# LBM-EPFL/MaD

Measured on NVIDIA B200. Metric: voxels/sec scale-space+detect+describe(+match), higher is better.
Workload: dtype f32 grids, f64 line accumulation, u8 x u8 -> s32 matching

## Files before the change

include/mad_b200.h:

```cpp
#ifndef MAD_B200_H
#define MAD_B200_H

#include <stddef.h>
#include <stdint.h>

#ifdef __cplusplus
extern "C" {
#endif

#define MAD_OK 0
#define MAD_ERR_ARG (-1)
#define MAD_ERR_CUDA (-2)
#define MAD_ERR_CAPACITY (-3)
#define MAD_ERR_NODEVICE (-4)

#define MAD_MAX_ORI 36
#define MAD_DSC_LEN 1024
#define MAD_DSC_REFUSED (1 << 30)

typedef struct MadKeypoint {
    int32_t vox[3];
    int32_t oct;
    float off[3];
    float val;
    int32_t peak[3];
    int32_t accepted;
} MadKeypoint;

typedef struct MadOriented {
    int32_t kp;
    int16_t main_bin;
    int16_t sec_bin;
} MadOriented;

typedef struct MadZoneTable {
    int32_t n_zones;
    int32_t n_belts;
    const double* bounds;
    const int32_t* belt_first;
    const double* belt_phi;
    const void* fast;
} MadZoneTable;

#define MAD_ZONE_FAST_BYTES 2048
int mad_zone_fast_build(const MadZoneTable* zones_host, void* fast_out, void* stream);

const char* mad_last_error_string(void);
int mad_version(void);
int mad_device_info(int* sm_count, int* cc_major, int* cc_minor);

int mad_publish_small(const void* src_dev, void* dst_host_mapped, int bytes, void* stream);

int mad_copy_to_host(const void* src_dev, void* dst_host_mapped, long long bytes, int n_ctas, void* stream);

long long mad_launch_count(void);
int mad_profile_enable(int on);
int mad_profile_count(void);
int mad_profile_get(int i, const char** name, float* ms);
int mad_profile_reset(void);

int mad_grid_max(const float* grid, long long n, float* out_max_ord, void* stream);
float mad_grid_max_decode(unsigned int ord);
int mad_threshold_normalise(float* grid, long long n, float isovalue, float vmax, int divide, void* stream);
int mad_grid_bbox(const float* grid, int nx, int ny, int nz, int* bbox6, void* stream);
int mad_crop_pad3d(const float* in, int nx, int ny, int nz, int x0, int y0, int z0, int cx, int cy, int cz,
                   int pad, float* out, void* stream);

int mad_pad3d(const float* in, int nx, int ny, int nz, int pad, float* out, void* stream);

size_t mad_upsample_workspace_bytes(int bx, int by, int bz);
int mad_upsample_presmooth(const float* base, int bx, int by, int bz,
                           const double* gauss_w_host, int radius,
                           float* up, void* workspace, size_t workspace_bytes, void* stream);

size_t mad_log_gauss_workspace_bytes(int nx, int ny, int nz);
int mad_log_gauss(const float* grid, int nx, int ny, int nz,
                  const double* w0_host, const double* w2_host, int radius, float scale,
                  float* log_out, float* gauss_out, void* workspace, size_t workspace_bytes,
                  int exact_f64, void* stream);

int mad_gradient(const float* gauss, int nx, int ny, int nz, float* grad4, void* stream);
size_t mad_gradient_tiles(int nx, int ny, int nz);
int mad_gradient_mark(const MadKeypoint* kp, int n_kp, const int* dims_oct_host, int reach_oct0, int reach_oct1,
                      uint8_t* flags_oct0, uint8_t* flags_oct1, void* stream);
int mad_gradient_masked(const float* gauss, int nx, int ny, int nz, float* grad4, uint8_t* flags, void* stream);

int mad_detect(const float* log_grid, int nx, int ny, int nz, int oct, int border,
               float threshold, MadKeypoint* cand, int cap, int* count, void* stream);

size_t mad_sort_keypoints_workspace_bytes(int n);
int mad_sort_keypoints(const MadKeypoint* cand, int n, const int* dims_oct_host,
                       MadKeypoint* out, int* out_count,
                       void* workspace, size_t workspace_bytes, void* stream);

int mad_orient(const float* grad4_oct0, const float* grad4_oct1, const int* dims_oct_host,
               const MadKeypoint* kp, int n_kp, int r, const MadZoneTable* zones112_host,
               const double* r1_table, int lim_main, int lim_sec,
               int32_t* n_ori, int32_t* slots, void* stream);

size_t mad_compact_oriented_workspace_bytes(int n_kp);
int mad_compact_oriented(const int32_t* n_ori, const int32_t* slots, int n_kp,
                         MadOriented* oriented, int cap, int* out_count,
                         void* workspace, size_t workspace_bytes, void* stream);

int mad_describe(const float* grad4_oct0, const float* grad4_oct1, const int* dims_oct_host,
                 const MadKeypoint* kp, const MadOriented* oriented, int n_oriented, int r,
                 const MadZoneTable* zones16_host, const double* rf_table, const double* rf_inv_table,
                 int rf_zones, int16_t* dsc, void* stream);

typedef struct MadDscSet {
    const int16_t* dsc;
    const void* half;
    const int32_t* norm2;
    const uint8_t* u8;
    const float* rnorm;
    int32_t rows;
    int32_t rows_padded;
    int32_t max_entry;
    int32_t max_norm2;
} MadDscSet;

int mad_dsc_prepare(const int16_t* dsc, int rows, int rows_padded, int32_t* norm2, float* rnorm,
                    uint8_t* u8, int32_t* max_entry, int32_t* max_norm2, void* stream);
int mad_dsc_norms(const int16_t* dsc, int rows, int32_t* norm2, void* stream);
int mad_dsc_to_half(const int16_t* dsc, int rows, int rows_padded, void* half_out, void* stream);

int mad_match_segments(int M, int N, int impl);
int mad_match_count(const MadDscSet* hi, const MadDscSet* lo, double cc, int n_seg, int32_t* seg_count, int impl,
                    void* stream);
int mad_match_fill(const MadDscSet* hi, const MadDscSet* lo, double cc, int n_seg, const int64_t* seg_offset,
                   int32_t* pair_hi, int32_t* pair_lo, double* pair_score, int impl, void* stream);
size_t mad_exclusive_scan_workspace_bytes(int n);
int mad_exclusive_scan_i32_to_i64(const int32_t* in, int n, int64_t* out, int64_t* total,
                                  void* workspace, size_t workspace_bytes, void* stream);

int mad_match_pairs(const MadDscSet* hi, const MadDscSet* lo, double cc, uint64_t* cand_key, int32_t* cand_dot,
                    uint64_t cap, uint64_t* count, void* stream);
size_t mad_match_pairs_finish_workspace_bytes(long long n);
int mad_match_pairs_finish(const uint64_t* cand_key, const int32_t* cand_dot, long long n, int hi_rows, int lo_rows,
                           const int32_t* hi_n2, const int32_t* lo_n2, int32_t* pair_hi, int32_t* pair_lo,
                           double* pair_score, void* workspace, size_t workspace_bytes, void* stream);
int mad_match_pairs_finish_dot(const uint64_t* cand_key, const int32_t* cand_dot, long long n, int hi_rows, int lo_rows,
                               int32_t* pair_hi, int32_t* pair_lo, int32_t* pair_dot, void* workspace, size_t workspace_bytes,
                               void* stream);

size_t mad_match_topk_workspace_bytes(int M, int N, int k, int impl);
int mad_match_topk(const MadDscSet* hi, const MadDscSet* lo, int k, int lo_index_base,
                   int32_t* topk_idx, double* topk_score, void* workspace, size_t workspace_bytes,
                   int impl, void* stream);
#define MAD_TOPK_INCOMPLETE (-2)
int mad_topk_merge(const int32_t* idx_in, const double* score_in, int G, int M, int k,
                   int32_t* idx_out, double* score_out, void* stream);

int mad_mark_used(const int32_t* idx, long long n, uint8_t* used, void* stream);
int mad_repeatability(const int32_t* pair_hi, const int32_t* pair_lo, const double* pair_score, long long n_pairs,
                      const double* hi_subv, const double* lo_subv, const int32_t* hi_meta, const int32_t* lo_meta,
                      const double* rf_table, const double* rf_inv_table, int rf_zones,
                      const double* hi_cloud, int n_hi_cloud, const double* lo_sorted, const int32_t* cell_start,
                      const uint32_t* near_bits, const double* grid_org_host, const int* grid_dims_host,
                      double dist, double* results, void* stream);

int mad_density_splat(const double* xyz, const double* mass, int n_atoms, const double* min_host, double voxelsp,
                      int margin, int px, int py, int pz, double* grid, void* stream);
int mad_normalise_f64(double* grid, long long n, void* scratch8, void* stream);
int mad_conv_full_f64(const double* in, long long outer, int n, long long inner, const double* w_dev, int radius,
                      void* out, int out_is_f32, void* stream);

size_t mad_box_scores_workspace_bytes(int ex, int ey, int ez);
int mad_box_scores(const float* g1, int nx1, int ny1, int nz1, const float* g2, int nx2, int ny2, int nz2,
                   const int* box_host, float isovalue, double* out8, void* workspace, size_t workspace_bytes,
                   void* stream);
int mad_grid_count_gt(const float* grid, long long n, float thr, unsigned long long* out, void* stream);
int mad_mask_with(float* g1, int nx1, int ny1, int nz1, const float* g2, int nx2, int ny2, int nz2,
                  const int* shift_host, const int* lo_host, const int* hi_host, void* stream);
int mad_refine_rigid(const float* grad4, int nx, int ny, int nz, const double* px, const double* py, const double* pz,
                     double voxsp, const double* init, const double* center, const double* max_dist, int n_problems,
                     int n_atoms, int n_steps, double max_step, double min_step, double* coords_out, double* meta_out,
                     void* stream);

#ifdef __cplusplus
}
#endif
#endif
```

mad_b200/_lib.py:

```python
import ctypes as C
import os

import numpy as np

HERE = os.path.dirname(os.path.abspath(__file__))
LIB_PATH = os.path.join(HERE, "libmad_b200.so")


class MadError(RuntimeError):
    pass


if not os.path.exists(LIB_PATH):
    raise ImportError(
        "mad_b200: %s is missing -- build the CUDA library first (python -m mad_b200.build). "
        "There is no CPU fallback." % LIB_PATH)

lib = C.CDLL(LIB_PATH)

KEYPOINT_DTYPE = np.dtype([("vox", "<i4", 3), ("oct", "<i4"), ("off", "<f4", 3), ("val", "<f4"),
                           ("peak", "<i4", 3), ("accepted", "<i4")])
ORIENTED_DTYPE = np.dtype([("kp", "<i4"), ("main", "<i2"), ("sec", "<i2")])
assert KEYPOINT_DTYPE.itemsize == 48 and ORIENTED_DTYPE.itemsize == 8
MAX_ORI = 36
DSC_LEN = 1024
DSC_REFUSED = 1 << 30
TOPK_INCOMPLETE = -2
TOPK_MAX = 32
ZONE_FAST_BYTES = 2048


class MadZoneTable(C.Structure):
    _fields_ = [("n_zones", C.c_int32), ("n_belts", C.c_int32), ("bounds", C.c_void_p),
                ("belt_first", C.c_void_p), ("belt_phi", C.c_void_p), ("fast", C.c_void_p)]


class MadDscSet(C.Structure):
    _fields_ = [("dsc", C.c_void_p), ("half", C.c_void_p), ("norm2", C.c_void_p), ("u8", C.c_void_p),
                ("rnorm", C.c_void_p), ("rows", C.c_int32), ("rows_padded", C.c_int32), ("max_entry", C.c_int32),
                ("max_norm2", C.c_int32)]


_P = C.c_void_p
_I = C.c_int
_SZ = C.c_size_t

SIGNATURES = {
    "mad_last_error_string": (C.c_char_p, []),
    "mad_version": (_I, []),
    "mad_device_info": (_I, [C.POINTER(_I), C.POINTER(_I), C.POINTER(_I)]),
    "mad_launch_count": (C.c_longlong, []),
    "mad_profile_enable": (_I, [_I]),
    "mad_profile_count": (_I, []),
    "mad_profile_get": (_I, [_I, C.POINTER(C.c_char_p), C.POINTER(C.c_float)]),
    "mad_profile_reset": (_I, []),
    "mad_publish_small": (_I, [_P, _P, _I, _P]),
    "mad_copy_to_host": (_I, [_P, _P, C.c_longlong, _I, _P]),
    "mad_zone_fast_build": (_I, [C.POINTER(MadZoneTable), _P, _P]),
    "mad_grid_max": (_I, [_P, C.c_longlong, _P, _P]),
    "mad_grid_max_decode": (C.c_float, [C.c_uint]),
    "mad_threshold_normalise": (_I, [_P, C.c_longlong, C.c_float, C.c_float, _I, _P]),
    "mad_grid_bbox": (_I, [_P, _I, _I, _I, _P, _P]),
    "mad_crop_pad3d": (_I, [_P, _I, _I, _I, _I, _I, _I, _I, _I, _I, _I, _P, _P]),
    "mad_pad3d": (_I, [_P, _I, _I, _I, _I, _P, _P]),
    "mad_upsample_workspace_bytes": (_SZ, [_I, _I, _I]),
    "mad_upsample_presmooth": (_I, [_P, _I, _I, _I, _P, _I, _P, _P, _SZ, _P]),
    "mad_log_gauss_workspace_bytes": (_SZ, [_I, _I, _I]),
    "mad_log_gauss": (_I, [_P, _I, _I, _I, _P, _P, _I, C.c_float, _P, _P, _P, _SZ, _I, _P]),
    "mad_gradient": (_I, [_P, _I, _I, _I, _P, _P]),
    "mad_gradient_tiles": (_SZ, [_I, _I, _I]),
    "mad_gradient_mark": (_I, [_P, _I, _P, _I, _I, _P, _P, _P]),
    "mad_gradient_masked": (_I, [_P, _I, _I, _I, _P, _P, _P]),
    "mad_detect": (_I, [_P, _I, _I, _I, _I, _I, C.c_float, _P, _I, _P, _P]),
    "mad_sort_keypoints_workspace_bytes": (_SZ, [_I]),
    "mad_sort_keypoints": (_I, [_P, _I, _P, _P, _P, _P, _SZ, _P]),
    "mad_orient": (_I, [_P, _P, _P, _P, _I, _I, C.POINTER(MadZoneTable), _P, _I, _I, _P, _P, _P]),
    "mad_compact_oriented_workspace_bytes": (_SZ, [_I]),
    "mad_compact_oriented": (_I, [_P, _P, _I, _P, _I, _P, _P, _SZ, _P]),
    "mad_describe": (_I, [_P, _P, _P, _P, _P, _I, _I, C.POINTER(MadZoneTable), _P, _P, _I, _P, _P]),
    "mad_dsc_prepare": (_I, [_P, _I, _I, _P, _P, _P, _P, _P, _P]),
    "mad_match_pairs": (_I, [C.POINTER(MadDscSet), C.POINTER(MadDscSet), C.c_double, _P, _P, C.c_uint64, _P, _P]),
    "mad_match_pairs_finish_workspace_bytes": (_SZ, [C.c_longlong]),
    "mad_match_pairs_finish": (_I, [_P, _P, C.c_longlong, _I, _I, _P, _P, _P, _P, _P, _P, _SZ, _P]),
    "mad_match_pairs_finish_dot": (_I, [_P, _P, C.c_longlong, _I, _I, _P, _P, _P, _P, _SZ, _P]),
    "mad_dsc_norms": (_I, [_P, _I, _P, _P]),
    "mad_dsc_to_half": (_I, [_P, _I, _I, _P, _P]),
    "mad_match_segments": (_I, [_I, _I, _I]),
    "mad_match_count": (_I, [C.POINTER(MadDscSet), C.POINTER(MadDscSet), C.c_double, _I, _P, _I, _P]),
    "mad_match_fill": (_I, [C.POINTER(MadDscSet), C.POINTER(MadDscSet), C.c_double, _I, _P, _P, _P, _P, _I, _P]),
    "mad_exclusive_scan_workspace_bytes": (_SZ, [_I]),
    "mad_exclusive_scan_i32_to_i64": (_I, [_P, _I, _P, _P, _P, _SZ, _P]),
    "mad_match_topk_workspace_bytes": (_SZ, [_I, _I, _I, _I]),
    "mad_match_topk": (_I, [C.POINTER(MadDscSet), C.POINTER(MadDscSet), _I, _I, _P, _P, _P, _SZ, _I, _P]),
    "mad_topk_merge": (_I, [_P, _P, _I, _I, _I, _P, _P, _P]),
    "mad_density_splat": (_I, [_P, _P, _I, _P, C.c_double, _I, _I, _I, _I, _P, _P]),
    "mad_normalise_f64": (_I, [_P, C.c_longlong, _P, _P]),
    "mad_conv_full_f64": (_I, [_P, C.c_longlong, _I, C.c_longlong, _P, _I, _P, _I, _P]),
    "mad_mark_used": (_I, [_P, C.c_longlong, _P, _P]),
    "mad_repeatability": (_I, [_P, _P, _P, C.c_longlong, _P, _P, _P, _P, _P, _P, _I, _P, _I, _P, _P, _P, _P, _P,
                               C.c_double, _P, _P]),
    "mad_box_scores_workspace_bytes": (_SZ, [_I, _I, _I]),
    "mad_box_scores": (_I, [_P, _I, _I, _I, _P, _I, _I, _I, _P, C.c_float, _P, _P, _SZ, _P]),
    "mad_grid_count_gt": (_I, [_P, C.c_longlong, C.c_float, _P, _P]),
    "mad_mask_with": (_I, [_P, _I, _I, _I, _P, _I, _I, _I, _P, _P, _P, _P]),
    "mad_refine_rigid": (_I, [_P, _I, _I, _I, _P, _P, _P, C.c_double, _P, _P, _P, _I, _I, _I, C.c_double, C.c_double,
                              _P, _P, _P]),
}

for _name, (_res, _args) in SIGNATURES.items():
    _f = getattr(lib, _name)
    _f.restype = _res
    _f.argtypes = _args


def last_error():
    s = lib.mad_last_error_string()
    return s.decode() if s else ""


def check(rc, what):
    if rc != 0:
        raise MadError("%s failed with status %d: %s" % (what, rc, last_error()))


def call(name, *args):
    check(getattr(lib, name)(*args), name)
```

mad_b200/csrc/api.cu:

```cuda
#include <stdarg.h>
#include <string.h>

#include "common.cuh"
#include "match_common.cuh"

static thread_local char g_err[512] = "";

void mad_set_error(const char* fmt, ...) {
    va_list ap;
    va_start(ap, fmt);
    vsnprintf(g_err, sizeof(g_err), fmt, ap);
    va_end(ap);
}

int mad_sm_count() {
    static int cached = 0;
    if (!cached) {
        int dev = 0, n = 0;
        if (cudaGetDevice(&dev) == cudaSuccess &&
            cudaDeviceGetAttribute(&n, cudaDevAttrMultiProcessorCount, dev) == cudaSuccess && n > 0)
            cached = n;
        else
            return 148;
    }
    return cached;
}

#include <atomic>
#include <mutex>
#include <vector>
namespace {
struct ProfRec { const char* name; cudaEvent_t a, b; };
std::atomic<long long> g_launches{0};
std::atomic<int> g_prof_on{0};
std::mutex g_prof_mu;
std::vector<ProfRec> g_prof;
}

MadProfScope::MadProfScope(const char* name, cudaStream_t stream) : slot(-1), st(stream) {
    g_launches.fetch_add(1, std::memory_order_relaxed);
    if (!g_prof_on.load(std::memory_order_relaxed)) return;
    ProfRec r;
    r.name = name;
    if (cudaEventCreate(&r.a) != cudaSuccess || cudaEventCreate(&r.b) != cudaSuccess) return;
    cudaEventRecord(r.a, st);
    std::lock_guard<std::mutex> lk(g_prof_mu);
    g_prof.push_back(r);
    slot = (int)g_prof.size() - 1;
}
MadProfScope::~MadProfScope() {
    if (slot < 0) return;
    std::lock_guard<std::mutex> lk(g_prof_mu);
    cudaEventRecord(g_prof[slot].b, st);
}

extern "C" long long mad_launch_count(void) { return g_launches.load(); }
extern "C" int mad_profile_enable(int on) {
    g_prof_on.store(on ? 1 : 0);
    return MAD_OK;
}
extern "C" int mad_profile_count(void) {
    std::lock_guard<std::mutex> lk(g_prof_mu);
    return (int)g_prof.size();
}
extern "C" int mad_profile_get(int i, const char** name, float* ms) {
    std::lock_guard<std::mutex> lk(g_prof_mu);
    MAD_CHECK_ARG(name && ms && i >= 0 && i < (int)g_prof.size());
    MAD_CUDA(cudaEventSynchronize(g_prof[i].b));
    MAD_CUDA(cudaEventElapsedTime(ms, g_prof[i].a, g_prof[i].b));
    *name = g_prof[i].name;
    return MAD_OK;
}
extern "C" int mad_profile_reset(void) {
    std::lock_guard<std::mutex> lk(g_prof_mu);
    for (auto& r : g_prof) { cudaEventDestroy(r.a); cudaEventDestroy(r.b); }
    g_prof.clear();
    return MAD_OK;
}

extern "C" const char* mad_last_error_string(void) { return g_err; }
extern "C" int mad_version(void) { return 100; }

extern "C" int mad_device_info(int* sm_count, int* cc_major, int* cc_minor) {
    MAD_CHECK_ARG(sm_count && cc_major && cc_minor);
    int dev = 0;
    MAD_CUDA(cudaGetDevice(&dev));
    MAD_CUDA(cudaDeviceGetAttribute(sm_count, cudaDevAttrMultiProcessorCount, dev));
    MAD_CUDA(cudaDeviceGetAttribute(cc_major, cudaDevAttrComputeCapabilityMajor, dev));
    MAD_CUDA(cudaDeviceGetAttribute(cc_minor, cudaDevAttrComputeCapabilityMinor, dev));
    return MAD_OK;
}

int mad_check_descriptor_sets(const MadDscSet* hi, const MadDscSet* lo, const char* who) {
    if (hi->max_entry >= MAD_DSC_REFUSED || lo->max_entry >= MAD_DSC_REFUSED) {
        mad_set_error("%s: not a descriptor set (a negative entry, or a squared norm >= 2^31)", who);
        return MAD_ERR_ARG;
    }
    return MAD_OK;
}

static bool fp16_exact(const MadDscSet* hi, const MadDscSet* lo) {
    return hi->max_entry >= 0 && lo->max_entry >= 0 && hi->max_entry <= 2048 && lo->max_entry <= 2048 &&
           hi->max_norm2 >= 0 && lo->max_norm2 >= 0 && (double)hi->max_norm2 * (double)lo->max_norm2 <= 281474976710656.0;
}

static int check_sets(const MadDscSet* hi, const MadDscSet* lo, int impl) {
    MAD_CHECK_ARG(hi && lo && hi->rows >= 0 && lo->rows >= 0);
    MAD_CHECK_ARG(impl == 0 || impl == 1 || impl == 2);
    if (hi->rows == 0 || lo->rows == 0) return MAD_OK;
    MAD_CHECK_ARG(hi->norm2 && lo->norm2);
    const int rc = mad_check_descriptor_sets(hi, lo, "mad_match");
    if (rc != MAD_OK) return rc;
    if (impl == 1) {
        MAD_CHECK_ARG(hi->dsc && lo->dsc);
    } else {
        if (impl == 2) MAD_CHECK_ARG(hi->half && lo->half);
        if (impl == 2 && !fp16_exact(hi, lo)) {
            mad_set_error("mad_match: the fp16 kernel (impl = 2) is exact only for entries in [0, 2048] and max |hi|^2 * max "
                          "|lo|^2 <= 2^48 (here max entry %d / %d, max |.|^2 %d / %d; -1 = not known): use impl = 1",
                          hi->max_entry, lo->max_entry, hi->max_norm2, lo->max_norm2);
            return MAD_ERR_ARG;
        }
        if (impl == 0) MAD_CHECK_ARG(hi->u8 && lo->u8 && lo->rnorm);
        MAD_CHECK_ARG(hi->rows_padded >= hi->rows && hi->rows_padded % 128 == 0);
        MAD_CHECK_ARG(lo->rows_padded >= lo->rows && lo->rows_padded % 128 == 0);
        if (impl == 0 && (hi->max_entry > 255 || lo->max_entry > 255)) {
            mad_set_error("mad_match: descriptor entries up to %d do not fit the uint8 kernel (use impl = 2)",
                          hi->max_entry > lo->max_entry ? hi->max_entry : lo->max_entry);
            return MAD_ERR_ARG;
        }
    }
    return MAD_OK;
}

static int run_match(const MadDscSet* hi, const MadDscSet* lo, double cc, int mode, int S, int32_t* seg_count,
                     const int64_t* seg_offset, int32_t* pair_hi, int32_t* pair_lo, double* pair_score, int k, int base,
                     int32_t* topk_idx, double* topk_score, int impl, cudaStream_t st) {
    if (impl == 1)
        return mad_match_simt(hi->dsc, hi->rows, lo->dsc, lo->rows, hi->norm2, lo->norm2, cc, mode, S, seg_count, seg_offset,
                              pair_hi, pair_lo, pair_score, k, base, topk_idx, topk_score, st);
    return mad_match_tc(hi->half, hi->rows, hi->rows_padded, lo->half, lo->rows, lo->rows_padded, hi->norm2, lo->norm2, cc,
                        mode, S, seg_count, seg_offset, pair_hi, pair_lo, pair_score, k, base, topk_idx, topk_score, st);
}

extern "C" int mad_match_segments(int M, int N, int impl) {
    return impl == 0 ? mad_match_u8_segments(M, N) : mad_match_tc_segments(M, N);
}

static int check_segments(const MadDscSet* hi, const MadDscSet* lo, int n_seg) {
    const int n_tiles = (int)mad_ceil_div(lo->rows, 128);
    MAD_CHECK_ARG(n_seg >= 1 && n_seg <= (n_tiles > 0 ? n_tiles : 1));
    (void)hi;
    return MAD_OK;
}

extern "C" int mad_match_count(const MadDscSet* hi, const MadDscSet* lo, double cc, int n_seg, int32_t* seg_count,
                               int impl, void* stream) {
    if (impl == 0) {
        mad_set_error("%s: impl 0 (the one-pass uint8 tcgen05 kernel) has no count/fill form -- call mad_match_pairs + "
                      "mad_match_pairs_finish; count/fill serve impl 1 (SIMT check) and 2 (fp16 tcgen05)", "mad_match_count");
        return MAD_ERR_ARG;
    }
    int rc = check_sets(hi, lo, impl);
    if (rc != MAD_OK) return rc;
    if (hi->rows == 0) return MAD_OK;
    MAD_CHECK_ARG(seg_count && n_seg >= 1);
    if (lo->rows == 0) {
        MAD_CUDA(cudaMemsetAsync(seg_count, 0, sizeof(int32_t) * (size_t)hi->rows * n_seg, (cudaStream_t)stream));
        return MAD_OK;
    }
    rc = check_segments(hi, lo, n_seg);
    if (rc != MAD_OK) return rc;
    return run_match(hi, lo, cc, 0, n_seg, seg_count, nullptr, nullptr, nullptr, nullptr, 0, 0, nullptr, nullptr, impl,
                     (cudaStream_t)stream);
}

extern "C" int mad_match_fill(const MadDscSet* hi, const MadDscSet* lo, double cc, int n_seg, const int64_t* seg_offset,
                              int32_t* pair_hi, int32_t* pair_lo, double* pair_score, int impl, void* stream) {
    if (impl == 0) {
        mad_set_error("%s: impl 0 (the one-pass uint8 tcgen05 kernel) has no count/fill form -- call mad_match_pairs + "
                      "mad_match_pairs_finish; count/fill serve impl 1 (SIMT check) and 2 (fp16 tcgen05)", "mad_match_fill");
        return MAD_ERR_ARG;
    }
    int rc = check_sets(hi, lo, impl);
    if (rc != MAD_OK) return rc;
    if (hi->rows == 0 || lo->rows == 0) return MAD_OK;
    MAD_CHECK_ARG(seg_offset && pair_hi && pair_lo && pair_score);
    rc = check_segments(hi, lo, n_seg);
    if (rc != MAD_OK) return rc;
    return run_match(hi, lo, cc, 1, n_seg, nullptr, seg_offset, pair_hi, pair_lo, pair_score, 0, 0, nullptr, nullptr, impl,
                     (cudaStream_t)stream);
}

static int u8_lists_per_segment(int k) { return k <= 8 ? 3 : 2; }
static int topk_lists(int M, int N, int k, int impl) {
    return impl == 0 ? u8_lists_per_segment(k) * mad_match_u8_segments_topk(M, N) : mad_match_segments(M, N, impl);
}

static size_t topk_part_workspace_bytes(int M, int N, int k, int impl) {
    const int S = topk_lists(M, N, k, impl);
    if (S <= 1 || M <= 0) return 256;
    return mad_align_up((size_t)S * M * k * sizeof(int32_t), 256) + mad_align_up((size_t)S * M * k * sizeof(double), 256);
}

static int topk_tail_rows(int M, int k, int impl) {
    if (impl != 0 || k > 8 || getenv("MAD_TOPK_NO_TAIL")) return 0;
    const int per_wave = mad_sm_count() / 2;
    const int pairs = (int)mad_ceil_div(M, 256);
    if (per_wave <= 0 || pairs <= per_wave) return 0;
    const int tail = pairs % per_wave;
    if (tail == 0 || 2 * tail > per_wave) return 0;
    return M - (pairs - tail) * 256;
}

extern "C" size_t mad_match_topk_workspace_bytes(int M, int N, int k, int impl) {
    const int tail = topk_tail_rows(M, k, impl);
    if (tail <= 0) return topk_part_workspace_bytes(M, N, k, impl);
    return std::max(topk_part_workspace_bytes(M - tail, N, k, impl), topk_part_workspace_bytes(tail, N, k, impl));
}

static int topk_part(const MadDscSet* hi, const MadDscSet* lo, int k, int lo_index_base, int32_t* topk_idx, double* topk_score,
                     void* workspace, size_t workspace_bytes, int impl, cudaStream_t st) {
    const int M = hi->rows;
    const int S = topk_lists(M, lo->rows, k, impl);
    auto run_topk = [&](int lists, int32_t* oi, double* os) {
        const int segs = impl == 0 ? lists / u8_lists_per_segment(k) : lists;
        if (impl == 0)
            return mad_match_u8_topk(hi->u8, hi->rows, hi->rows_padded, lo->u8, lo->rows, lo->rows_padded, hi->norm2,
                                     lo->norm2, lo->rnorm, segs, k, lo_index_base, oi, os, st);
        return run_match(hi, lo, 0.0, 2, segs, nullptr, nullptr, nullptr, nullptr, nullptr, k, lo_index_base, oi, os, impl, st);
    };
    if (S == 1) return run_topk(1, topk_idx, topk_score);
    MAD_CHECK_ARG(workspace && workspace_bytes >= topk_part_workspace_bytes(M, lo->rows, k, impl));
    int32_t* pidx = reinterpret_cast<int32_t*>(workspace);
    double* pscore = reinterpret_cast<double*>(reinterpret_cast<char*>(workspace) +
                                               mad_align_up((size_t)S * M * k * sizeof(int32_t), 256));
    int rc = run_topk(S, pidx, pscore);
    if (rc != MAD_OK) return rc;
    return mad_topk_merge_launch(pidx, pscore, S, M, k, topk_idx, topk_score, st);
}

extern "C" int mad_match_topk(const MadDscSet* hi, const MadDscSet* lo, int k, int lo_index_base, int32_t* topk_idx,
                              double* topk_score, void* workspace, size_t workspace_bytes, int impl, void* stream) {
    int rc = check_sets(hi, lo, impl);
    if (rc != MAD_OK) return rc;
    MAD_CHECK_ARG(k >= 1 && k <= MAD_TOPK_MAX);
    if (hi->rows == 0) return MAD_OK;
    MAD_CHECK_ARG(topk_idx && topk_score);
    cudaStream_t st = (cudaStream_t)stream;
    const int M = hi->rows;
    if (lo->rows == 0) {
        MAD_CUDA(cudaMemsetAsync(topk_idx, 0xFF, sizeof(int32_t) * (size_t)M * k, st));
        return mad_topk_merge_launch(topk_idx, topk_score, 0, M, k, topk_idx, topk_score, st);
    }
    const int tail = topk_tail_rows(M, k, impl);
    if (tail <= 0) return topk_part(hi, lo, k, lo_index_base, topk_idx, topk_score, workspace, workspace_bytes, impl, st);
    const int M0 = M - tail;
    MadDscSet a = *hi, b = *hi;
    a.rows = M0;
    a.rows_padded = M0;
    b.rows = tail;
    b.rows_padded = hi->rows_padded - M0;
    b.dsc = hi->dsc ? hi->dsc + (size_t)M0 * MAD_DSC_LEN : nullptr;
    b.u8 = hi->u8 ? hi->u8 + (size_t)M0 * MAD_DSC_LEN : nullptr;
    b.norm2 = hi->norm2 + M0;
    b.rnorm = hi->rnorm ? hi->rnorm + M0 : nullptr;
    rc = topk_part(&a, lo, k, lo_index_base, topk_idx, topk_score, workspace, workspace_bytes, impl, st);
    if (rc != MAD_OK) return rc;
    return topk_part(&b, lo, k, lo_index_base, topk_idx + (size_t)M0 * k, topk_score + (size_t)M0 * k, workspace, workspace_bytes,
                     impl, st);
}

namespace {
__global__ void publish_small_kernel(const unsigned int* __restrict__ src, volatile unsigned int* dst, int n_words) {
    for (int i = threadIdx.x; i < n_words; i += blockDim.x) dst[i] = src[i];
    __threadfence_system();
}
}

extern "C" int mad_publish_small(const void* src_dev, void* dst_host_mapped, int bytes, void* stream) {
    MAD_CHECK_ARG(src_dev && dst_host_mapped && bytes > 0 && bytes <= 4096 && bytes % 4 == 0);
    MAD_CHECK_ARG((reinterpret_cast<uintptr_t>(src_dev) & 3) == 0 && (reinterpret_cast<uintptr_t>(dst_host_mapped) & 3) == 0);
    MAD_PROF("publish_small_kernel", stream);
    publish_small_kernel<<<1, 64, 0, (cudaStream_t)stream>>>(static_cast<const unsigned int*>(src_dev),
                                                             static_cast<volatile unsigned int*>(dst_host_mapped), bytes / 4);
    MAD_LAUNCH_OK();
    return MAD_OK;
}

namespace {
__global__ void __launch_bounds__(256)
copy_to_host_kernel(const uint4* __restrict__ src, uint4* __restrict__ dst, long long n16, const unsigned char* __restrict__ src_tail,
                    unsigned char* __restrict__ dst_tail, int n_tail) {
    const long long stride = (long long)gridDim.x * blockDim.x;
    for (long long i = blockIdx.x * (long long)blockDim.x + threadIdx.x; i < n16; i += stride) {
        const uint4 v = __ldcs(src + i);
        __stcs(dst + i, v);
    }
    if (blockIdx.x == 0 && (int)threadIdx.x < n_tail) dst_tail[threadIdx.x] = src_tail[threadIdx.x];
}
}

extern "C" int mad_copy_to_host(const void* src_dev, void* dst_host_mapped, long long bytes, int n_ctas, void* stream) {
    MAD_CHECK_ARG(src_dev && dst_host_mapped && bytes > 0 && n_ctas >= 1 && n_ctas <= 1024);
    MAD_CHECK_ARG((reinterpret_cast<uintptr_t>(src_dev) & 15) == 0 && (reinterpret_cast<uintptr_t>(dst_host_mapped) & 15) == 0);
    const long long n16 = bytes / 16;
    const int n_tail = (int)(bytes - n16 * 16);
    const unsigned char* s8 = static_cast<const unsigned char*>(src_dev);
    unsigned char* d8 = static_cast<unsigned char*>(dst_host_mapped);
    MAD_PROF("copy_to_host_kernel", stream);
    copy_to_host_kernel<<<n_ctas, 256, 0, (cudaStream_t)stream>>>(static_cast<const uint4*>(src_dev), static_cast<uint4*>(dst_host_mapped),
                                                                  n16, s8 + n16 * 16, d8 + n16 * 16, n_tail);
    MAD_LAUNCH_OK();
    return MAD_OK;
}
```

mad_b200/csrc/match_common.cuh:

```cuda
#pragma once
#include <math.h>
#include "common.cuh"

#define MAD_TOPK_MAX 32

__host__ __device__ __forceinline__ double mad_score(int dot, double n2a, double n2b) {
    const double p = n2a * n2b;
    return p > 0.0 ? (double)dot / sqrt(p) : 0.0;
}

__host__ __device__ __forceinline__ void mad_topk_insert(double* bs, int* bi, int k, double s, int id) {
    const double ls = bs[k - 1];
    const int li = bi[k - 1];
    if (!(s > ls || (s == ls && (li < 0 || id < li)))) return;
    int q = k - 1;
    while (q > 0) {
        const double ps = bs[q - 1];
        const int pi = bi[q - 1];
        if (s > ps || (s == ps && (pi < 0 || id < pi))) { bs[q] = ps; bi[q] = pi; --q; }
        else break;
    }
    bs[q] = s;
    bi[q] = id;
}

__host__ __device__ __forceinline__ bool mad_topk_before(double s, int id, double ps, int pi) {
    return s > ps || (s == ps && (pi < 0 || id < pi));
}

__device__ __forceinline__ void mad_top8_insert(double (&bs)[8], int (&bi)[8], double s, int id) {
    bool c[8];
#pragma unroll
    for (int q = 0; q < 8; ++q) c[q] = mad_topk_before(s, id, bs[q], bi[q]);
#pragma unroll
    for (int q = 7; q >= 1; --q) {
        bs[q] = c[q - 1] ? bs[q - 1] : (c[q] ? s : bs[q]);
        bi[q] = c[q - 1] ? bi[q - 1] : (c[q] ? id : bi[q]);
    }
    bs[0] = c[0] ? s : bs[0];
    bi[0] = c[0] ? id : bi[0];
}

static __device__ __noinline__ bool mad_score_before_nl(int d, int n, int id, int pd, int pn, int pi, double n2a) {
    return mad_topk_before(mad_score(d, n2a, (double)n), id, mad_score(pd, n2a, (double)pn), pi);
}
__device__ __forceinline__ bool mad_score32_before(float s, int d, int n, int id, float ps, int pd, int pn, int pi, double n2a) {
    if (pi < 0) return true;
    const float tol = 4e-6f * fmaxf(s, ps);
    if (s > ps + tol) return true;
    if (s < ps - tol) return false;
    return mad_score_before_nl(d, n, id, pd, pn, pi, n2a);
}

__device__ __forceinline__ void mad_top8f_insert(float (&ts)[8], int (&td)[8], int (&tn)[8], int (&bi)[8], bool active, float s,
                                                 int d, int n, int id, double n2a) {
    bool c[8];
    bool amb = false;
#pragma unroll
    for (int q = 0; q < 8; ++q) {
        const float ps = ts[q];
        const bool empty = bi[q] < 0;
        const float tol = 4e-6f * fmaxf(s, ps);
        const bool gt = s > ps + tol, lt = s < ps - tol;
        c[q] = active && (empty || gt);
        amb |= active && !empty && !gt && !lt;
    }
    if (__any_sync(0xFFFFFFFFu, amb)) {
#pragma unroll
        for (int q = 0; q < 8; ++q) c[q] = active && mad_score32_before(s, d, n, id, ts[q], td[q], tn[q], bi[q], n2a);
    }
#pragma unroll
    for (int q = 7; q >= 1; --q) {
        ts[q] = c[q - 1] ? ts[q - 1] : (c[q] ? s : ts[q]);
        td[q] = c[q - 1] ? td[q - 1] : (c[q] ? d : td[q]);
        tn[q] = c[q - 1] ? tn[q - 1] : (c[q] ? n : tn[q]);
        bi[q] = c[q - 1] ? bi[q - 1] : (c[q] ? id : bi[q]);
    }
    ts[0] = c[0] ? s : ts[0];
    td[0] = c[0] ? d : td[0];
    tn[0] = c[0] ? n : tn[0];
    bi[0] = c[0] ? id : bi[0];
}

__device__ __forceinline__ void mad_st_release_cta(volatile int* p, int v) {
    asm volatile("st.release.cta.shared::cta.s32 [%0], %1;" ::"r"((uint32_t)__cvta_generic_to_shared((const void*)p)), "r"(v) : "memory");
}
__device__ __forceinline__ int mad_ld_acquire_cta(volatile int* p) {
    int v;
    asm volatile("ld.acquire.cta.shared::cta.s32 %0, [%1];" : "=r"(v) : "r"((uint32_t)__cvta_generic_to_shared((const void*)p)) : "memory");
    return v;
}

__device__ __forceinline__ uint32_t mad_select32(const uint32_t (&v)[32], int j) {
    uint32_t a[16];
#pragma unroll
    for (int i = 0; i < 16; ++i) a[i] = (j & 1) ? v[2 * i + 1] : v[2 * i];
    uint32_t b[8];
#pragma unroll
    for (int i = 0; i < 8; ++i) b[i] = (j & 2) ? a[2 * i + 1] : a[2 * i];
    uint32_t c[4];
#pragma unroll
    for (int i = 0; i < 4; ++i) c[i] = (j & 4) ? b[2 * i + 1] : b[2 * i];
    const uint32_t d0 = (j & 8) ? c[1] : c[0], d1 = (j & 8) ? c[3] : c[2];
    return (j & 16) ? d1 : d0;
}

#define MAD_MATCH_SEG_TILE 256

int mad_check_descriptor_sets(const MadDscSet* hi, const MadDscSet* lo, const char* who);

int mad_match_simt(const int16_t* hi, int M, const int16_t* lo, int N, const int32_t* hi_n2, const int32_t* lo_n2,
                   double cc, int mode, int S, int32_t* seg_count, const int64_t* seg_offset, int32_t* pair_hi,
                   int32_t* pair_lo, double* pair_score, int k, int lo_index_base, int32_t* topk_idx,
                   double* topk_score, cudaStream_t st);

int mad_match_tc_segments(int M, int N);
int mad_match_tc(const void* hi_half, int M, int M_pad, const void* lo_half, int N, int N_pad,
                 const int32_t* hi_n2, const int32_t* lo_n2, double cc, int mode, int S, int32_t* seg_count,
                 const int64_t* seg_offset, int32_t* pair_hi, int32_t* pair_lo, double* pair_score, int k,
                 int lo_index_base, int32_t* topk_idx, double* topk_score, cudaStream_t st);
int mad_topk_merge_launch(const int32_t* idx_in, const double* score_in, int G, int M, int k, int32_t* idx_out,
                          double* score_out, cudaStream_t st);

int mad_match_u8_segments(int M, int N);
int mad_match_u8_segments_topk(int M, int N);
int mad_match_u8_pairs(const void* hi_u8, int M, int M_pad, const void* lo_u8, int N, int N_pad, const int32_t* hi_n2,
                       const int32_t* lo_n2, const float* lo_rnorm, double cc, unsigned long long* cand_key,
                       int32_t* cand_dot, unsigned long long cap, unsigned long long* count, cudaStream_t st);
int mad_match_u8_topk(const void* hi_u8, int M, int M_pad, const void* lo_u8, int N, int N_pad, const int32_t* hi_n2,
                      const int32_t* lo_n2, const float* lo_rnorm, int S, int k, int lo_index_base, int32_t* topk_idx,
                      double* topk_score, cudaStream_t st);
```

mad_b200/csrc/match_prep.cu:

```cuda
#include <cub/cub.cuh>

#include "common.cuh"
#include "match_common.cuh"

namespace {

__global__ void __launch_bounds__(256)
dsc_prepare_kernel(const int16_t* __restrict__ dsc, int rows, int rows_padded, int32_t* __restrict__ norm2,
                   float* __restrict__ rnorm, uint8_t* __restrict__ u8, int32_t* __restrict__ max_entry,
                   int32_t* __restrict__ max_norm2) {
    const int row = (int)((blockIdx.x * (long long)blockDim.x + threadIdx.x) >> 5);
    const int lane = threadIdx.x & 31;
    if (row >= rows_padded) return;
    long long acc = 0;
    int mx = 0;
    uint32_t packed[8];
    if (row < rows) {
        const uint4* src = reinterpret_cast<const uint4*>(dsc + (long long)row * MAD_DSC_LEN + lane * 32);
#pragma unroll
        for (int q = 0; q < 4; ++q) {
            const uint4 v = __ldg(src + q);
            const uint32_t w[4] = {v.x, v.y, v.z, v.w};
#pragma unroll
            for (int h = 0; h < 4; ++h) {
                const int e0 = (int)(int16_t)(w[h] & 0xFFFFu), e1 = (int)(int16_t)(w[h] >> 16);
                acc += (long long)e0 * e0 + (long long)e1 * e1;
                mx = max(mx, max(e0, e1));
                if (e0 < 0 || e1 < 0) mx = MAD_DSC_REFUSED;
                const uint32_t b0 = (uint32_t)min(max(e0, 0), 255), b1 = (uint32_t)min(max(e1, 0), 255);
                const int slot = q * 8 + h * 2;
                if ((slot & 3) == 0) packed[slot >> 2] = b0 | (b1 << 8);
                else packed[slot >> 2] |= (b0 << 16) | (b1 << 24);
            }
        }
    } else {
#pragma unroll
        for (int q = 0; q < 8; ++q) packed[q] = 0;
    }
    if (u8) {
        uint4* dst = reinterpret_cast<uint4*>(u8 + (long long)row * MAD_DSC_LEN + lane * 32);
        dst[0] = make_uint4(packed[0], packed[1], packed[2], packed[3]);
        dst[1] = make_uint4(packed[4], packed[5], packed[6], packed[7]);
    }
#pragma unroll
    for (int o = 16; o > 0; o >>= 1) {
        acc += __shfl_xor_sync(0xFFFFFFFFu, acc, o);
        mx = max(mx, __shfl_xor_sync(0xFFFFFFFFu, mx, o));
    }
    if (lane == 0) {
        if (acc > 0x7FFFFFFFLL) mx = MAD_DSC_REFUSED;
        if (row < rows) norm2[row] = (int32_t)acc;
        rnorm[row] = acc > 0 ? (float)(1.0 / sqrt((double)acc)) : 0.f;
        if (mx > 0) atomicMax(max_entry, mx);
        if (max_norm2 && acc > 0) atomicMax(max_norm2, (int32_t)min(acc, 0x7FFFFFFFLL));
    }
}

__global__ void pairs_finish_kernel(const unsigned long long* __restrict__ key, const int32_t* __restrict__ dot,
                                    long long n, unsigned long long lo_rows, const int32_t* __restrict__ hi_n2,
                                    const int32_t* __restrict__ lo_n2,
                                    int32_t* __restrict__ pair_hi, int32_t* __restrict__ pair_lo,
                                    double* __restrict__ score) {
    const long long i = blockIdx.x * (long long)blockDim.x + threadIdx.x;
    if (i >= n) return;
    const unsigned long long k = key[i];
    const int row = (int)(k / lo_rows), col = (int)(k % lo_rows);
    pair_hi[i] = row;
    pair_lo[i] = col;
    score[i] = mad_score(dot[i], (double)__ldg(hi_n2 + row), (double)__ldg(lo_n2 + col));
}

__global__ void pairs_finish_dot_kernel(const unsigned long long* __restrict__ key, const int32_t* __restrict__ dot, long long n,
                                        unsigned long long lo_rows, int32_t* __restrict__ pair_hi, int32_t* __restrict__ pair_lo,
                                        int32_t* __restrict__ pair_dot) {
    const long long i = blockIdx.x * (long long)blockDim.x + threadIdx.x;
    if (i >= n) return;
    const unsigned long long k = key[i];
    pair_hi[i] = (int)(k / lo_rows);
    pair_lo[i] = (int)(k % lo_rows);
    pair_dot[i] = dot[i];
}

__global__ void zero_u64_kernel(unsigned long long* p) { *p = 0ull; }

struct FinishLayout {
    size_t key_off, dot_off, cub_off, cub_bytes, total;
};

FinishLayout finish_layout(long long n) {
    FinishLayout L;
    const size_t nn = (size_t)(n > 0 ? n : 1);
    L.key_off = 0;
    L.dot_off = mad_align_up(nn * sizeof(unsigned long long), 256);
    L.cub_off = L.dot_off + mad_align_up(nn * sizeof(int32_t), 256);
    size_t b = 0;
    cub::DeviceRadixSort::SortPairs(nullptr, b, (const unsigned long long*)nullptr, (unsigned long long*)nullptr,
                                    (const int32_t*)nullptr, (int32_t*)nullptr, (int)nn, 0, 64);
    L.cub_bytes = mad_align_up(b, 256);
    L.total = L.cub_off + L.cub_bytes;
    return L;
}

}

extern "C" int mad_dsc_prepare(const int16_t* dsc, int rows, int rows_padded, int32_t* norm2, float* rnorm,
                               uint8_t* u8, int32_t* max_entry, int32_t* max_norm2, void* stream) {
    MAD_CHECK_ARG(rows >= 0 && rows_padded >= rows);
    if (rows_padded == 0) return MAD_OK;
    MAD_CHECK_ARG((rows == 0 || dsc) && norm2 && rnorm && max_entry);
    MAD_CHECK_ARG((reinterpret_cast<uintptr_t>(dsc) & 15) == 0 && (reinterpret_cast<uintptr_t>(u8) & 15) == 0);
    MAD_PROF("dsc_prepare_kernel", stream);
    dsc_prepare_kernel<<<(unsigned)mad_ceil_div((long long)rows_padded * 32, 256), 256, 0, (cudaStream_t)stream>>>(
        dsc, rows, rows_padded, norm2, rnorm, u8, max_entry, max_norm2);
    MAD_LAUNCH_OK();
    return MAD_OK;
}

extern "C" int mad_match_pairs(const MadDscSet* hi, const MadDscSet* lo, double cc, uint64_t* cand_key, int32_t* cand_dot,
                               uint64_t cap, uint64_t* count, void* stream) {
    MAD_CHECK_ARG(hi && lo && count && hi->rows >= 0 && lo->rows >= 0);
    cudaStream_t st = (cudaStream_t)stream;
    {
        MAD_PROF("zero_u64_kernel", st);
        zero_u64_kernel<<<1, 1, 0, st>>>(reinterpret_cast<unsigned long long*>(count));
        MAD_LAUNCH_OK();
    }
    if (hi->rows == 0 || lo->rows == 0) return MAD_OK;
    MAD_CHECK_ARG(hi->u8 && lo->u8 && hi->norm2 && lo->norm2 && lo->rnorm && cand_key && cand_dot);
    MAD_CHECK_ARG(hi->rows_padded >= hi->rows && hi->rows_padded % 128 == 0);
    MAD_CHECK_ARG(lo->rows_padded >= lo->rows && lo->rows_padded % 128 == 0);
    int rc = mad_check_descriptor_sets(hi, lo, "mad_match_pairs");
    if (rc != MAD_OK) return rc;
    if (hi->max_entry > 255 || lo->max_entry > 255) {
        mad_set_error("mad_match_pairs: descriptor entries up to %d do not fit the uint8 tensor-core operand "
                      "(use mad_match_count/mad_match_fill with impl = 2 or 1)",
                      hi->max_entry > lo->max_entry ? hi->max_entry : lo->max_entry);
        return MAD_ERR_ARG;
    }
    return mad_match_u8_pairs(hi->u8, hi->rows, hi->rows_padded, lo->u8, lo->rows, lo->rows_padded, hi->norm2, lo->norm2,
                              lo->rnorm, cc, reinterpret_cast<unsigned long long*>(cand_key), cand_dot,
                              (unsigned long long)cap, reinterpret_cast<unsigned long long*>(count), st);
}

extern "C" size_t mad_match_pairs_finish_workspace_bytes(long long n) { return finish_layout(n).total; }

static int pairs_finish_impl(const uint64_t* cand_key, const int32_t* cand_dot, long long n, int hi_rows, int lo_rows,
                             const int32_t* hi_n2, const int32_t* lo_n2, int32_t* pair_hi, int32_t* pair_lo, double* pair_score,
                             int32_t* pair_dot, void* workspace, size_t workspace_bytes, void* stream);

extern "C" int mad_match_pairs_finish(const uint64_t* cand_key, const int32_t* cand_dot, long long n, int hi_rows,
                                      int lo_rows, const int32_t* hi_n2, const int32_t* lo_n2, int32_t* pair_hi, int32_t* pair_lo,
                                      double* pair_score, void* workspace, size_t workspace_bytes, void* stream) {
    MAD_CHECK_ARG(n >= 0 && n < (1LL << 31));
    if (n == 0) return MAD_OK;
    MAD_CHECK_ARG(hi_n2 && lo_n2 && pair_score);
    return pairs_finish_impl(cand_key, cand_dot, n, hi_rows, lo_rows, hi_n2, lo_n2, pair_hi, pair_lo, pair_score, nullptr, workspace,
                             workspace_bytes, stream);
}

extern "C" int mad_match_pairs_finish_dot(const uint64_t* cand_key, const int32_t* cand_dot, long long n, int hi_rows, int lo_rows,
                                          int32_t* pair_hi, int32_t* pair_lo, int32_t* pair_dot, void* workspace,
                                          size_t workspace_bytes, void* stream) {
    MAD_CHECK_ARG(n >= 0 && n < (1LL << 31));
    if (n == 0) return MAD_OK;
    MAD_CHECK_ARG(pair_dot);
    return pairs_finish_impl(cand_key, cand_dot, n, hi_rows, lo_rows, nullptr, nullptr, pair_hi, pair_lo, nullptr, pair_dot, workspace,
                             workspace_bytes, stream);
}

static int pairs_finish_impl(const uint64_t* cand_key, const int32_t* cand_dot, long long n, int hi_rows, int lo_rows,
                             const int32_t* hi_n2, const int32_t* lo_n2, int32_t* pair_hi, int32_t* pair_lo, double* pair_score,
                             int32_t* pair_dot, void* workspace, size_t workspace_bytes, void* stream) {
    MAD_CHECK_ARG(cand_key && cand_dot && pair_hi && pair_lo && workspace && hi_rows > 0 && lo_rows > 0);
    const FinishLayout L = finish_layout(n);
    MAD_CHECK_ARG(workspace_bytes >= L.total);
    cudaStream_t st = (cudaStream_t)stream;
    char* ws = reinterpret_cast<char*>(workspace);
    unsigned long long* key_sorted = reinterpret_cast<unsigned long long*>(ws + L.key_off);
    int32_t* dot_sorted = reinterpret_cast<int32_t*>(ws + L.dot_off);
    int key_bits = 1;
    while (key_bits < 64 && (1ULL << key_bits) < (unsigned long long)hi_rows * (unsigned long long)lo_rows) ++key_bits;
    size_t b = L.cub_bytes;
    {
        MAD_PROF("cub_radix_sort_pairs", st);
        MAD_CUDA(cub::DeviceRadixSort::SortPairs(ws + L.cub_off, b, reinterpret_cast<const unsigned long long*>(cand_key),
                                                 key_sorted, cand_dot, dot_sorted, (int)n, 0, key_bits, st));
    }
    MAD_PROF("pairs_finish_kernel", st);
    if (pair_dot)
        pairs_finish_dot_kernel<<<(unsigned)mad_ceil_div(n, 256), 256, 0, st>>>(key_sorted, dot_sorted, n, (unsigned long long)lo_rows, pair_hi,
                                                                               pair_lo, pair_dot);
    else
        pairs_finish_kernel<<<(unsigned)mad_ceil_div(n, 256), 256, 0, st>>>(key_sorted, dot_sorted, n, (unsigned long long)lo_rows, hi_n2, lo_n2,
                                                                           pair_hi, pair_lo, pair_score);
    MAD_LAUNCH_OK();
    return MAD_OK;
}
```

mad_b200/csrc/match_u8.cu:

```cuda
#include <cuda.h>
#include <stdlib.h>

#include <type_traits>

#include "common.cuh"
#include "match_common.cuh"

namespace {

constexpr int BM = 128;
constexpr int BN = 128;
constexpr int BKB = 128;
constexpr int UKB = 32;
constexpr int KBLOCKS = MAD_DSC_LEN / BKB;
constexpr int STAGES = 5;
constexpr int STAGES2 = 10;
constexpr int ACCS = 4;
constexpr uint32_t KB_BYTES = BM * BKB;
constexpr uint32_t A_BYTES = KBLOCKS * KB_BYTES;
constexpr int EPI_WARPS = 8;
constexpr int THREADS = 128 + 32 * EPI_WARPS + 64;
constexpr uint32_t TMEM_COLS = 512;
constexpr unsigned long long MAD_MATCH_TIMEOUT_COUNT = 1ull << 62;
constexpr int STG = 96;
constexpr size_t STG_BYTES = (size_t)EPI_WARPS * STG * (sizeof(unsigned long long) + sizeof(int));
constexpr size_t RB_BYTES = (size_t)2 * 2 * 256 * sizeof(float);
constexpr size_t THR_BYTES = 512;
constexpr int TOP_SLOTS = 2;
constexpr int TOP_LOCAL_TILES = 4;
constexpr unsigned long long TOP_INVALID = ~0ull;
static_assert((size_t)EPI_WARPS * 2 * 32 * TOP_SLOTS * sizeof(unsigned long long) <= STG_BYTES, "TOP8 slots fit the staging area");
constexpr size_t SMEM_BYTES = 1024 + A_BYTES + (size_t)STAGES * KB_BYTES + STG_BYTES + RB_BYTES + 512 + THR_BYTES;
static_assert(SMEM_BYTES <= 232448, "shared memory budget of one sm_100 CTA");

__device__ __forceinline__ uint32_t smem_u32(const void* p) { return (uint32_t)__cvta_generic_to_shared(p); }
__device__ __forceinline__ void mbar_init(uint32_t bar, uint32_t count) {
    asm volatile("mbarrier.init.shared::cta.b64 [%0], %1;" ::"r"(bar), "r"(count) : "memory");
}
__device__ __forceinline__ void mbar_expect_tx(uint32_t bar, uint32_t bytes) {
    asm volatile("mbarrier.arrive.expect_tx.shared::cta.b64 _, [%0], %1;" ::"r"(bar), "r"(bytes) : "memory");
}
__device__ __forceinline__ void mbar_arrive(uint32_t bar) {
    asm volatile("mbarrier.arrive.shared::cta.b64 _, [%0];" ::"r"(bar) : "memory");
}
__device__ __forceinline__ void mbar_wait(uint32_t bar, uint32_t parity) {
    uint32_t done;
    do {
        asm volatile(
            "{\n\t.reg .pred p;\n\t"
            "mbarrier.try_wait.parity.shared::cta.b64 p, [%1], %2;\n\t"
            "selp.u32 %0, 1, 0, p;\n\t}"
            : "=r"(done)
            : "r"(bar), "r"(parity)
            : "memory");
    } while (!done);
}
__device__ __forceinline__ void tma_load_2d(uint32_t dst, const CUtensorMap* map, uint32_t bar, int c0, int c1) {
    asm volatile(
        "cp.async.bulk.tensor.2d.shared::cluster.global.mbarrier::complete_tx::bytes [%0], [%1, {%3, %4}], [%2];"
        ::"r"(dst), "l"(reinterpret_cast<uint64_t>(map)), "r"(bar), "r"(c0), "r"(c1)
        : "memory");
}
constexpr uint32_t kPeerBitMask = 0xFEFFFFFFu;
__device__ __forceinline__ uint32_t cluster_ctarank() {
    uint32_t r;
    asm volatile("mov.u32 %0, %%cluster_ctarank;" : "=r"(r));
    return r;
}
__device__ __forceinline__ void cluster_sync_all() {
    asm volatile("barrier.cluster.arrive.release.aligned;" ::: "memory");
    asm volatile("barrier.cluster.wait.acquire.aligned;" ::: "memory");
}
__device__ __forceinline__ void tma_load_2d_2sm(uint32_t dst, const CUtensorMap* map, uint32_t bar, int c0, int c1) {
    asm volatile(
        "cp.async.bulk.tensor.2d.cta_group::2.shared::cluster.global.mbarrier::complete_tx::bytes [%0], [%1, {%3, %4}], [%2];"
        ::"r"(dst), "l"(reinterpret_cast<uint64_t>(map)), "r"(bar & kPeerBitMask), "r"(c0), "r"(c1)
        : "memory");
}
__device__ __forceinline__ void mbar_arrive_leader(uint32_t bar) {
    asm volatile("mbarrier.arrive.shared::cluster.b64 _, [%0];" ::"r"(bar & kPeerBitMask) : "memory");
}
__device__ __forceinline__ void umma_commit_pair(uint32_t bar) {
    asm volatile("tcgen05.commit.cta_group::2.mbarrier::arrive::one.shared::cluster.multicast::cluster.b64 [%0], %1;"
                 ::"r"(bar), "h"((uint16_t)3) : "memory");
}
__device__ __forceinline__ void umma_i8_pair(uint32_t d_tmem, uint64_t a_desc, uint64_t b_desc, uint32_t idesc, uint32_t accumulate) {
    asm volatile(
        "{\n\t.reg .pred p;\n\t"
        "setp.ne.b32 p, %4, 0;\n\t"
        "tcgen05.mma.cta_group::2.kind::i8 [%0], %1, %2, %3, p;\n\t}"
        ::"r"(d_tmem), "l"(a_desc), "l"(b_desc), "r"(idesc), "r"(accumulate)
        : "memory");
}
__device__ __forceinline__ void umma_commit(uint32_t bar) {
    asm volatile("tcgen05.commit.cta_group::1.mbarrier::arrive::one.shared::cluster.b64 [%0];" ::"r"(bar) : "memory");
}
__device__ __forceinline__ void umma_i8(uint32_t d_tmem, uint64_t a_desc, uint64_t b_desc, uint32_t idesc, uint32_t accumulate) {
    asm volatile(
        "{\n\t.reg .pred p;\n\t"
        "setp.ne.b32 p, %4, 0;\n\t"
        "tcgen05.mma.cta_group::1.kind::i8 [%0], %1, %2, %3, p;\n\t}"
        ::"r"(d_tmem), "l"(a_desc), "l"(b_desc), "r"(idesc), "r"(accumulate)
        : "memory");
}
__device__ __forceinline__ void tmem_ld32(uint32_t taddr, uint32_t (&v)[32]) {
    asm volatile(
        "tcgen05.ld.sync.aligned.32x32b.x32.b32 "
        "{%0, %1, %2, %3, %4, %5, %6, %7, %8, %9, %10, %11, %12, %13, %14, %15, "
        "%16, %17, %18, %19, %20, %21, %22, %23, %24, %25, %26, %27, %28, %29, %30, %31}, [%32];"
        : "=r"(v[0]), "=r"(v[1]), "=r"(v[2]), "=r"(v[3]), "=r"(v[4]), "=r"(v[5]), "=r"(v[6]), "=r"(v[7]),
          "=r"(v[8]), "=r"(v[9]), "=r"(v[10]), "=r"(v[11]), "=r"(v[12]), "=r"(v[13]), "=r"(v[14]), "=r"(v[15]),
          "=r"(v[16]), "=r"(v[17]), "=r"(v[18]), "=r"(v[19]), "=r"(v[20]), "=r"(v[21]), "=r"(v[22]), "=r"(v[23]),
          "=r"(v[24]), "=r"(v[25]), "=r"(v[26]), "=r"(v[27]), "=r"(v[28]), "=r"(v[29]), "=r"(v[30]), "=r"(v[31])
        : "r"(taddr)
        : "memory");
}
__device__ __forceinline__ uint32_t tmem_ld1(uint32_t taddr) {
    uint32_t x;
    asm volatile("tcgen05.ld.sync.aligned.32x32b.x1.b32 {%0}, [%1];" : "=r"(x) : "r"(taddr) : "memory");
    return x;
}
__device__ __forceinline__ void tmem_ld_wait() { asm volatile("tcgen05.wait::ld.sync.aligned;" ::: "memory"); }
__device__ __forceinline__ void tc_fence_before() { asm volatile("tcgen05.fence::before_thread_sync;" ::: "memory"); }
__device__ __forceinline__ void tc_fence_after() { asm volatile("tcgen05.fence::after_thread_sync;" ::: "memory"); }

__device__ __forceinline__ uint64_t umma_smem_desc(uint32_t saddr) {
    uint64_t d = 0;
    d |= (uint64_t)((saddr & 0x3FFFFu) >> 4);
    d |= (uint64_t)1 << 16;
    d |= (uint64_t)(1024u >> 4) << 32;
    d |= (uint64_t)1 << 46;
    d |= (uint64_t)2 << 61;
    return d;
}
constexpr uint32_t kIdesc = (2u << 4) | ((uint32_t)(BN >> 3) << 17) | ((uint32_t)(BM >> 4) << 24);
constexpr uint32_t kIdescPair = (2u << 4) | ((uint32_t)((2 * BN) >> 3) << 17) | ((uint32_t)((2 * BM) >> 4) << 24);

struct U8Args {
    int M, N, S;
    int tiles_per_seg;
    const int32_t* hi_n2;
    const int32_t* lo_n2;
    const float* lo_rnorm;
    double cc;
    unsigned long long* cand_key;
    int32_t* cand_dot;
    unsigned long long cap;
    unsigned long long* count;
    int k, lo_index_base;
    int local_tiles;
    int dbg;
    int32_t* topk_idx;
    double* topk_score;
};

__device__ unsigned long long g_top_dbg[8];

enum { MODE_PAIRS = 0, MODE_TOPK = 1, MODE_TOP8 = 2 };

template <int MODE, int NCTA>
__global__ void __launch_bounds__(THREADS, 1)
match_u8_kernel(const __grid_constant__ CUtensorMap map_hi, const __grid_constant__ CUtensorMap map_lo, U8Args a) {
    constexpr int TN = (NCTA == 2) ? 2 * BN : BN;
    constexpr int NACC = (int)TMEM_COLS / TN;
    constexpr int NSTAGE = STAGES;
    constexpr uint32_t SB = KB_BYTES;
    extern __shared__ uint8_t smem_raw[];
    const uint32_t raw = smem_u32(smem_raw);
    const uint32_t base = (raw + 1023u) & ~1023u;
    uint8_t* gen = smem_raw + (base - raw);
    const uint32_t b_ring = base + A_BYTES;
    constexpr uint32_t STG_OFF = A_BYTES + STAGES * KB_BYTES;
    unsigned long long* stg_key = reinterpret_cast<unsigned long long*>(gen + STG_OFF);
    int* stg_dot = reinterpret_cast<int*>(gen + STG_OFF + EPI_WARPS * STG * sizeof(unsigned long long));
    float* s_rb = reinterpret_cast<float*>(gen + STG_OFF + (uint32_t)STG_BYTES);
    constexpr uint32_t BAR_OFF = STG_OFF + (uint32_t)(STG_BYTES + RB_BYTES);
    const uint32_t bars = base + BAR_OFF;
    auto full_bar = [&](int s) { return bars + 8u * s; };
    auto empty_bar = [&](int s) { return bars + 8u * (NSTAGE + s); };
    auto tfull_bar = [&](int q) { return bars + 8u * (2 * NSTAGE + q); };
    auto tempty_bar = [&](int q) { return bars + 8u * (2 * NSTAGE + ACCS + q); };
    const uint32_t a_bar = bars + 8u * (2 * NSTAGE + 2 * ACCS);
    uint32_t* tmem_slot = reinterpret_cast<uint32_t*>(gen + BAR_OFF + 8 * (2 * NSTAGE + 2 * ACCS + 1));
    volatile int* s_half = reinterpret_cast<volatile int*>(gen + BAR_OFF + 8 * (2 * NSTAGE + 2 * ACCS + 2));
    volatile int* s_done = s_half + 2 * EPI_WARPS;
    static_assert(8 * (2 * STAGES + 2 * ACCS + 2) + 3 * EPI_WARPS * sizeof(int) <= 512, "misc shared region");
    volatile unsigned long long* top_slots = reinterpret_cast<volatile unsigned long long*>(gen + STG_OFF);
    volatile float* s_thr8 = reinterpret_cast<volatile float*>(gen + BAR_OFF + 512);

    const int warp = threadIdx.x >> 5, lane = threadIdx.x & 31;
    const uint32_t rank = (NCTA == 2) ? cluster_ctarank() : 0u;
    const int m0 = blockIdx.x * BM;
    const int seg = blockIdx.y;
    const int n_tiles_total = (a.N + TN - 1) / TN;
    const int t_begin = seg * a.tiles_per_seg;
    const int t_end = min(n_tiles_total, t_begin + a.tiles_per_seg);

    if (threadIdx.x == 0) {
        for (int s = 0; s < NSTAGE; ++s) { mbar_init(full_bar(s), 1); mbar_init(empty_bar(s), 1); }
        for (int q = 0; q < NACC; ++q) { mbar_init(tfull_bar(q), 1); mbar_init(tempty_bar(q), NCTA == 2 ? 16 : 4); }
        mbar_init(a_bar, 1);
        asm volatile("fence.mbarrier_init.release.cluster;" ::: "memory");
    }
    if (threadIdx.x < 3 * EPI_WARPS) s_half[threadIdx.x] = 0;
    volatile float* s_thr = reinterpret_cast<volatile float*>(gen + STG_OFF);
    if (MODE == MODE_TOPK && threadIdx.x < 2 * BM) s_thr[threadIdx.x] = -1.f;
    if (MODE == MODE_TOP8) {
        for (int i = threadIdx.x; i < EPI_WARPS * 2 * 32 * TOP_SLOTS; i += THREADS) top_slots[i] = TOP_INVALID;
        if (threadIdx.x < BM) s_thr8[threadIdx.x] = -1.f;
    }
    if (NCTA == 2) cluster_sync_all();
    if (warp == 2) {
        if (NCTA == 2) {
            asm volatile("tcgen05.alloc.cta_group::2.sync.aligned.shared::cta.b32 [%0], %1;" ::"r"(smem_u32(tmem_slot)), "n"(TMEM_COLS) : "memory");
            asm volatile("tcgen05.relinquish_alloc_permit.cta_group::2.sync.aligned;" ::: "memory");
        } else {
            asm volatile("tcgen05.alloc.cta_group::1.sync.aligned.shared::cta.b32 [%0], %1;" ::"r"(smem_u32(tmem_slot)), "n"(TMEM_COLS) : "memory");
            asm volatile("tcgen05.relinquish_alloc_permit.cta_group::1.sync.aligned;" ::: "memory");
        }
    }
    tc_fence_before();
    __syncthreads();
    tc_fence_after();
    const uint32_t tmem_base = *tmem_slot;

    if (warp == 0) {
        if (lane == 0) {
            if (NCTA == 2) {
                if (rank == 0) mbar_expect_tx(a_bar, 2 * A_BYTES);
                for (int kb = 0; kb < KBLOCKS; ++kb) tma_load_2d_2sm(base + kb * KB_BYTES, &map_hi, a_bar, kb * BKB, m0);
            } else {
                mbar_expect_tx(a_bar, A_BYTES);
                for (int kb = 0; kb < KBLOCKS; ++kb) tma_load_2d(base + kb * KB_BYTES, &map_hi, a_bar, kb * BKB, m0);
            }
            int stage = 0;
            uint32_t phase = 0;
            for (int t = t_begin; t < t_end; ++t) {
                for (int kb = 0; kb < KBLOCKS; ++kb) {
                    mbar_wait(empty_bar(stage), phase ^ 1u);
                    if (NCTA == 2) {
                        if (rank == 0) mbar_expect_tx(full_bar(stage), 2 * KB_BYTES);
                        tma_load_2d_2sm(b_ring + stage * SB, &map_lo, full_bar(stage), kb * BKB, t * TN + (int)rank * BN);
                    } else {
                        mbar_expect_tx(full_bar(stage), KB_BYTES);
                        tma_load_2d(b_ring + stage * SB, &map_lo, full_bar(stage), kb * BKB, t * BN);
                    }
                    if (++stage == NSTAGE) { stage = 0; phase ^= 1u; }
                }
            }
        }
    } else if (warp == 1) {
        if (lane == 0 && rank == 0) {
            mbar_wait(a_bar, 0);
            tc_fence_after();
            int stage = 0;
            uint32_t phase = 0;
            int it = 0;
            for (int t = t_begin; t < t_end; ++t, ++it) {
                const int acc = it % NACC;
                const uint32_t acc_phase = (uint32_t)(it / NACC) & 1u;
                mbar_wait(tempty_bar(acc), acc_phase ^ 1u);
                tc_fence_after();
                const uint32_t d_tmem = tmem_base + (uint32_t)(acc * TN);
                for (int kb = 0; kb < KBLOCKS; ++kb) {
                    mbar_wait(full_bar(stage), phase);
                    tc_fence_after();
                    const uint64_t da = umma_smem_desc(base + kb * KB_BYTES);
                    const uint64_t db = umma_smem_desc(b_ring + stage * SB);
#pragma unroll
                    for (int kk = 0; kk < BKB / UKB; ++kk) {
                        if (NCTA == 2) umma_i8_pair(d_tmem, da + (uint64_t)(2 * kk), db + (uint64_t)(2 * kk), kIdescPair, (kb | kk) ? 1u : 0u);
                        else umma_i8(d_tmem, da + (uint64_t)(2 * kk), db + (uint64_t)(2 * kk), kIdesc, (kb | kk) ? 1u : 0u);
                    }
                    if (NCTA == 2) umma_commit_pair(empty_bar(stage)); else umma_commit(empty_bar(stage));
                    if (++stage == NSTAGE) { stage = 0; phase ^= 1u; }
                }
                if (NCTA == 2) umma_commit_pair(tfull_bar(acc)); else umma_commit(tfull_bar(acc));
            }
        }
    } else if (warp >= 2 && warp < 4 && MODE == MODE_PAIRS) {
        constexpr int HALF = STG / 2;
        const int e0 = (warp - 2) * 4;
        const double cc2 = a.cc * a.cc;
        int hi_n2_reg[4];
#pragma unroll
        for (int qq = 0; qq < 4; ++qq) hi_n2_reg[qq] = (m0 + qq * 32 + lane < a.M) ? __ldg(a.hi_n2 + m0 + qq * 32 + lane) : 0;
        for (long long spins = 0; spins < (1LL << 27); ++spins) {
            int done = 0;
            for (int e = e0; e < e0 + 4; ++e) done += mad_ld_acquire_cta(&s_done[e]);
            bool any = false;
            for (int e = e0; e < e0 + 4; ++e) {
                for (int h = 0; h < 2; ++h) {
                    const int n = mad_ld_acquire_cta(&s_half[2 * e + h]);
                    if (n <= 0) continue;
                    any = true;
                    const unsigned long long* hk = stg_key + e * STG + h * HALF;
                    const int* hd = stg_dot + e * STG + h * HALF;
                    unsigned long long ent[2];
                    int dot[2];
                    bool ok[2];
#pragma unroll
                    for (int k = 0; k < 2; ++k) {
                        const int i = lane + 32 * k;
                        ent[k] = (i < n) ? hk[i] : 0ull;
                        dot[k] = (i < n) ? hd[i] : 0;
                    }
                    __syncwarp();
                    if (lane == 0) mad_st_release_cta(&s_half[2 * e + h], 0);
                    int total = 0, pos[2];
                    const int qe = e & 3;
                    const int n2_q = qe == 0 ? hi_n2_reg[0] : (qe == 1 ? hi_n2_reg[1] : (qe == 2 ? hi_n2_reg[2] : hi_n2_reg[3]));
#pragma unroll
                    for (int k = 0; k < 2; ++k) {
                        ok[k] = false;
                        const unsigned low = (unsigned)ent[k];
                        const double n2r = (double)__shfl_sync(0xFFFFFFFFu, n2_q, (int)(low & 31u));
                        if (lane + 32 * k < n) {
                            const int row = m0 + qe * 32 + (int)(low & 31u);
                            const double n2c = (double)(unsigned)(ent[k] >> 32);
                            const double p = n2r * n2c, lhs = (double)dot[k] * (double)dot[k], rhs = cc2 * p;
                            if (p > 0.0 && a.cc > 0.0 && lhs > rhs * (1.0 + 1e-13)) ok[k] = true;
                            else if (p > 0.0 && a.cc > 0.0 && lhs < rhs * (1.0 - 1e-13)) ok[k] = false;
                            else ok[k] = mad_score(dot[k], n2r, n2c) > a.cc;
                            ent[k] = (unsigned long long)row * (unsigned long long)a.N + (unsigned long long)(low >> 5);
                        }
                        const unsigned m = __ballot_sync(0xFFFFFFFFu, ok[k]);
                        pos[k] = total + __popc(m & ((1u << lane) - 1u));
                        total += __popc(m);
                    }
                    if (total > 0) {
                        unsigned long long gb = 0;
                        if (lane == 0) gb = atomicAdd(a.count, (unsigned long long)total);
                        gb = __shfl_sync(0xFFFFFFFFu, gb, 0);
#pragma unroll
                        for (int k = 0; k < 2; ++k)
                            if (ok[k] && gb + pos[k] < a.cap) { a.cand_key[gb + pos[k]] = ent[k]; a.cand_dot[gb + pos[k]] = dot[k]; }
                    }
                }
            }
            if (!any) {
                if (done == 4) break;
                __nanosleep(200);
            }
            if (spins == (1LL << 27) - 1 && lane == 0) atomicExch(a.count, MAD_MATCH_TIMEOUT_COUNT);
        }
    } else if ((warp == 2 || warp == 3 || warp >= 4 + EPI_WARPS) && MODE == MODE_TOP8) {
        const int dq = warp < 4 ? warp - 2 : warp - (4 + EPI_WARPS) + 2;
        float ts[8];
        int td[8], tn[8], bi[8];
#pragma unroll
        for (int i = 0; i < 8; ++i) { ts[i] = 0.f; td[i] = 0; tn[i] = 1; bi[i] = -1; }
        const int row = m0 + 32 * dq + lane;
        const int n2a_i = row < a.M ? __ldg(a.hi_n2 + row) : 0;
        const float ra = n2a_i > 0 ? (float)(1.0 / sqrt((double)n2a_i)) : 0.f;
        bool timeout = false;
        for (long long spins = 0;; ++spins) {
            if (spins >= (1LL << 26)) { timeout = true; break; }
            const int done = mad_ld_acquire_cta(&s_done[dq]) + mad_ld_acquire_cta(&s_done[4 + dq]);
            bool any = false;
#pragma unroll 1
            for (int g = 0; g < 2; ++g) {
                const int e = g * 4 + dq;
#pragma unroll 1
                for (int h = 0; h < 2; ++h) {
                    const int tt = mad_ld_acquire_cta(&s_half[2 * e + h]);
                    if (tt <= 0) continue;
                    any = true;
                    const long long dc0 = (a.dbg & 32) ? clock64() : 0;
                    int n_ins = 0, n_stale = 0;
                    volatile unsigned long long* sl = top_slots + ((e * 2 + h) * 32 + lane) * TOP_SLOTS;
                    unsigned long long ent[TOP_SLOTS];
#pragma unroll
                    for (int u = 0; u < TOP_SLOTS; ++u) { ent[u] = sl[u]; sl[u] = TOP_INVALID; }
                    __syncwarp();
                    if (lane == 0) mad_st_release_cta(&s_half[2 * e + h], 0);
                    const int colbase = a.lo_index_base + (tt - 1) * TN;
                    bool changed = false;
#pragma unroll
                    for (int u = 0; u < TOP_SLOTS; ++u) {
                        const bool has = ent[u] != TOP_INVALID && !(a.dbg & 1);
                        if (!__any_sync(0xFFFFFFFFu, has)) continue;
                        const int dot = (int)(ent[u] >> 35), n2b = (int)((ent[u] >> 8) & 0x7FFFFFFull);
                        const int id = colbase + (int)(ent[u] & 0xFFull);
                        const bool nz = n2a_i > 0 && n2b > 0;
                        const float s32 = nz ? (float)dot * rsqrtf((float)n2b) * ra : 0.f;
                        const bool live = has && (bi[7] < 0 || s32 >= ts[7] * (1.f - 4e-6f));
                        if (!__any_sync(0xFFFFFFFFu, live)) { n_stale += has; continue; }
                        mad_top8f_insert(ts, td, tn, bi, live, s32, nz ? dot : 0, nz ? n2b : 1, id, (double)n2a_i);
                        changed |= live;
                        n_ins += live;
                        n_stale += has && !live;
                    }
                    if (a.dbg & 32) {
                        n_ins = __reduce_add_sync(0xFFFFFFFFu, n_ins);
                        n_stale = __reduce_add_sync(0xFFFFFFFFu, n_stale);
                        if (lane == 0) {
                            atomicAdd(&g_top_dbg[4], 1ull); atomicAdd(&g_top_dbg[5], (unsigned long long)(clock64() - dc0));
                            atomicAdd(&g_top_dbg[6], (unsigned long long)n_ins); atomicAdd(&g_top_dbg[7], (unsigned long long)n_stale);
                        }
                    }
                    if (changed && bi[7] >= 0) atomicMax(reinterpret_cast<int*>(const_cast<float*>(&s_thr8[dq * 32 + lane])), __float_as_int(fmaxf(ts[7] - 4e-6f, 0.f)));
                }
            }
            if (!any) {
                if (done == 2) break;
                __nanosleep(a.dbg & 16 ? 32 : (a.dbg & 64 ? 1000 : 300));
            }
        }
        if (row < a.M) {
            const long long o = ((long long)(seg * 3) * a.M + row) * a.k;
#pragma unroll
            for (int i = 0; i < 8; ++i)
                if (i < a.k) {
                    a.topk_idx[o + i] = timeout ? MAD_TOPK_INCOMPLETE : bi[i];
                    a.topk_score[o + i] = bi[i] < 0 ? -INFINITY : (td[i] == 0 ? 0.0 : mad_score(td[i], (double)n2a_i, (double)tn[i]));
                }
        }
    } else if (warp >= 4 && warp < 4 + EPI_WARPS) {
        const int q = warp & 3;
        const int ew = warp - 4;
        const int grp = ew >> 2;
        const int row = m0 + q * 32 + lane;
        const bool row_ok = row < a.M;
        const int n2a_i = row_ok ? a.hi_n2[row] : 0;
        const double n2a = (double)n2a_i;
        const float ra = n2a_i > 0 ? (float)(1.0 / sqrt(n2a)) : 0.f;
        const float thr_pairs = !row_ok ? INFINITY : (n2a_i > 0 ? ((float)a.cc - 4e-6f) / ra : (a.cc < 0.0 ? -INFINITY : INFINITY));
        unsigned long long* my_key = stg_key + ew * STG;
        int* my_dot = stg_dot + ew * STG;
        constexpr bool kTop = (MODE == MODE_TOPK || MODE == MODE_TOP8);
        constexpr int kList = (MODE == MODE_TOPK) ? MAD_TOPK_MAX : 1;
        double bs[kList];
        int bi[kList];
        float thr = -1.f;
        if (MODE == MODE_TOPK) {
#pragma unroll
            for (int i = 0; i < kList; ++i) { bs[i] = -INFINITY; bi[i] = -1; }
        }
        const int k_last = a.k - 1;
        int top_cnt = 0;
        float ls[8];
        int ld[8], ln[8], li[8];
        if (MODE == MODE_TOP8) {
#pragma unroll
            for (int i = 0; i < 8; ++i) { ls[i] = 0.f; ld[i] = 0; ln[i] = 1; li[i] = -1; }
        }
        auto flush_local = [&]() {
            if (li[7] >= 0) atomicMax(reinterpret_cast<int*>(const_cast<float*>(&s_thr8[q * 32 + lane])), __float_as_int(fmaxf(ls[7] - 4e-6f, 0.f)));
            if (row_ok) {
                const long long o = ((long long)(seg * 3 + 1 + grp) * a.M + row) * a.k;
#pragma unroll
                for (int i = 0; i < 8; ++i)
                    if (i < a.k) {
                        a.topk_idx[o + i] = li[i];
                        a.topk_score[o + i] = li[i] < 0 ? -INFINITY : (ld[i] == 0 ? 0.0 : mad_score(ld[i], n2a, (double)ln[i]));
                    }
            }
        };
        int stg_n = 0;
        constexpr int HALF = STG / 2;
        static_assert(HALF >= 32, "a half buffer must take one ballot round");
        int cur = 0;
        auto publish = [&](int n) {
            __syncwarp();
            if (n > 0) {
                if (lane == 0) {
                    mad_st_release_cta(&s_half[2 * ew + cur], n);
                    long long spins = 0;
                    while (mad_ld_acquire_cta(&s_half[2 * ew + (cur ^ 1)]) != 0 && ++spins < (1LL << 27)) __nanosleep(64);
                    if (spins >= (1LL << 27)) atomicExch(a.count, MAD_MATCH_TIMEOUT_COUNT);
                }
                cur ^= 1;
                __syncwarp();
            }
        };
        auto publish_top = [&](int t) {
            __syncwarp();
            if (lane == 0) {
                mad_st_release_cta(&s_half[2 * ew + cur], t + 1);
                long long spins = 0;
                const long long c0 = (a.dbg & 32) ? clock64() : 0;
                while (mad_ld_acquire_cta(&s_half[2 * ew + (cur ^ 1)]) != 0 && ++spins < (1LL << 26)) __nanosleep(32);
                if (a.dbg & 32) { atomicAdd(&g_top_dbg[1], (unsigned long long)(clock64() - c0)); atomicAdd(&g_top_dbg[2], 1ull); }
            }
            cur ^= 1;
            top_cnt = 0;
            __syncwarp();
        };
        constexpr bool kSplitCols = (NCTA == 2);
        constexpr int kStep = kSplitCols ? 1 : 2;
        const int c_lo = kSplitCols ? grp * BN : 0;
        float* my_rb = s_rb + grp * 2 * 256;
        const int gt = threadIdx.x - 128 - grp * 128;
        auto stage_rb = [&](int t, int buf) {
            if (gt < BN / 4) {
                const float4 r4 = __ldg(reinterpret_cast<const float4*>(a.lo_rnorm + (long long)t * TN + c_lo) + gt);
                reinterpret_cast<float4*>(my_rb + buf * 256)[gt] = r4;
                {
                    const int c = t * TN + c_lo + 4 * gt;
                    int4 n4;
                    n4.x = (c < a.N) ? __ldg(a.lo_n2 + c) : 0;
                    n4.y = (c + 1 < a.N) ? __ldg(a.lo_n2 + c + 1) : 0;
                    n4.z = (c + 2 < a.N) ? __ldg(a.lo_n2 + c + 2) : 0;
                    n4.w = (c + 3 < a.N) ? __ldg(a.lo_n2 + c + 3) : 0;
                    reinterpret_cast<int4*>(my_rb + buf * 256 + 128)[gt] = n4;
                }
            }
        };
        auto group_sync = [&]() { asm volatile("bar.sync %0, 128;" ::"r"(1 + grp) : "memory"); };
        const int t_first = t_begin + (kSplitCols ? 0 : grp);
        int it = kSplitCols ? 0 : grp;
        int par = 0;
        if (t_first < t_end) stage_rb(t_first, 0);
        auto tile_body = [&](auto local_tag, const int t, const int it, const int par) {
            const int acc = it % NACC;
            const uint32_t acc_phase = (uint32_t)(it / NACC) & 1u;
            const int n0 = t * TN;
            constexpr bool top_local = decltype(local_tag)::value;
            group_sync();
            if (t + kStep < t_end) stage_rb(t + kStep, par ^ 1);
            const float* rbt = my_rb + par * 256 - c_lo;
            mbar_wait(tfull_bar(acc), acc_phase);
            tc_fence_after();
            const uint32_t taddr = tmem_base + ((uint32_t)(q * 32) << 16) + (uint32_t)(acc * TN);
#pragma unroll 1
            for (int c0 = c_lo; c0 < c_lo + BN; c0 += 32) {
                uint32_t v[32];
                tmem_ld32(taddr + (uint32_t)c0, v);
                tmem_ld_wait();
                if (c0 == c_lo + BN - 32 && !(a.dbg & 4)) {
                    tc_fence_before();
                    __syncwarp();
                    if (lane == 0) {
                        if (NCTA == 2) mbar_arrive_leader(tempty_bar(acc)); else mbar_arrive(tempty_bar(acc));
                    }
                }
                float thr_eff = thr;
                if (MODE == MODE_TOPK && kSplitCols) thr_eff = fmaxf(thr, s_thr[(grp ^ 1) * BM + q * 32 + lane]);
                if (MODE == MODE_TOP8)
                    thr_eff = top_local ? (li[7] < 0 ? -1.f : ls[7] - 4e-6f) : s_thr8[q * 32 + lane];
                const float lim = kTop ? (row_ok && ra > 0.f ? thr_eff / ra : INFINITY) : thr_pairs;
                unsigned mask = 0;
#pragma unroll
                for (int j4 = 0; j4 < 8; ++j4) {
                    const float4 r4 = reinterpret_cast<const float4*>(rbt + c0)[j4];
                    const float rb[4] = {r4.x, r4.y, r4.z, r4.w};
#pragma unroll
                    for (int u = 0; u < 4; ++u) {
                        const float sc = (float)(int)v[4 * j4 + u] * rb[u];
                        const bool pass = kTop ? (sc >= lim) : (sc > lim);
                        mask |= (pass ? 1u : 0u) << (4 * j4 + u);
                    }
                }
                if (MODE == MODE_TOPK && row_ok && ra == 0.f) mask = (bi[k_last] < 0) ? 0xFFFFFFFFu : 0u;
                if (MODE == MODE_TOP8) {
                    if (row_ok && ra == 0.f) mask = (t == t_begin && c0 == 0) ? 0xFFu : 0u;
                    const int left = a.N - (n0 + c0);
                    if (left < 32) mask &= (left <= 0) ? 0u : ((1u << left) - 1u);
                    if (a.dbg & 2) mask = 0u;
                    if (top_local) {
                        for (;;) {
                            if (__ballot_sync(0xFFFFFFFFu, mask != 0u) == 0u) break;
                            const bool has = mask != 0u;
                            const int j = has ? __ffs(mask) - 1 : 0;
                            mask &= mask - 1;
                            const int dot = (int)mad_select32(v, j);
                            const int n2b = __float_as_int(rbt[c0 + j + 128]);
                            const bool nz = n2a_i > 0 && n2b > 0;
                            const float s32 = nz ? (float)dot * rbt[c0 + j] * ra : 0.f;
                            const bool live = has && (li[7] < 0 || s32 >= ls[7] * (1.f - 4e-6f));
                            if (__any_sync(0xFFFFFFFFu, live))
                                mad_top8f_insert(ls, ld, ln, li, live, s32, nz ? dot : 0, nz ? n2b : 1, a.lo_index_base + n0 + c0 + j, n2a);
                        }
                        continue;
                    }
                    const long long rc0 = (a.dbg & 32) ? clock64() : 0;
                    int n_rounds = 0;
                    for (;;) {
                        const unsigned b = __ballot_sync(0xFFFFFFFFu, mask != 0u);
                        if (b == 0u) break;
                        ++n_rounds;
                        if (__ballot_sync(0xFFFFFFFFu, mask != 0u && top_cnt == TOP_SLOTS) != 0u) publish_top(t);
                        if (mask) {
                            const int j = __ffs(mask) - 1;
                            mask &= mask - 1;
                            const unsigned long long dot = (unsigned long long)mad_select32(v, j);
                            const unsigned long long n2b = (unsigned long long)(unsigned)__float_as_int(rbt[c0 + j + 128]);
                            top_slots[((ew * 2 + cur) * 32 + lane) * TOP_SLOTS + top_cnt] = (dot << 35) | (n2b << 8) | (unsigned long long)(c0 + j);
                            ++top_cnt;
                        }
                    }
                    if ((a.dbg & 32) && lane == 0 && n_rounds) {
                        atomicAdd(&g_top_dbg[0], (unsigned long long)(clock64() - rc0));
                        atomicAdd(&g_top_dbg[3], (unsigned long long)n_rounds);
                    }
                } else if (kTop) {
                    while (mask) {
                        const int j = __ffs(mask) - 1;
                        mask &= mask - 1;
                        const int dot = (int)mad_select32(v, j);
                        const int col = n0 + c0 + j;
                        if (col < a.N) {
                            const int n2b = __float_as_int(rbt[c0 + j + 128]);
                            {
                                const double s = mad_score(dot, n2a, (double)n2b);
                                mad_topk_insert(bs, bi, a.k, s, a.lo_index_base + col);
                                thr = (bi[k_last] < 0) ? -1.f : (float)bs[k_last] - 4e-6f;
                                if (kSplitCols) s_thr[grp * BM + q * 32 + lane] = thr;
                            }
                        }
                    }
                } else {
                    const int left = a.N - (n0 + c0);
                    if (left < 32) mask &= (left <= 0) ? 0u : ((1u << left) - 1u);
                    const unsigned lt = (1u << lane) - 1u;
                    for (;;) {
                        const unsigned b = __ballot_sync(0xFFFFFFFFu, mask != 0u);
                        if (b == 0u) break;
                        const int nb = __popc(b);
                        if (stg_n + nb > HALF) { publish(stg_n); stg_n = 0; }
                        if (mask) {
                            const int j = __ffs(mask) - 1;
                            mask &= mask - 1;
                            const int p = cur * HALF + stg_n + __popc(b & lt);
                            my_key[p] = ((unsigned long long)(unsigned)__float_as_int(rbt[c0 + j + 128]) << 32) |
                                        (unsigned long long)(((unsigned)(n0 + c0 + j) << 5) | (unsigned)lane);
                            my_dot[p] = (int)mad_select32(v, j);
                        }
                        stg_n += nb;
                    }
                }
            }
            if (a.dbg & 4) {
                tc_fence_before();
                __syncwarp();
                if (lane == 0) { if (NCTA == 2) mbar_arrive_leader(tempty_bar(acc)); else mbar_arrive(tempty_bar(acc)); }
            }
            if (MODE == MODE_TOP8 && __ballot_sync(0xFFFFFFFFu, top_cnt > 0) != 0u) publish_top(t);
        };
        int t = t_first;
        if (MODE == MODE_TOP8) {
            for (int n = 0; n < a.local_tiles && t < t_end; ++n, t += kStep, it += kStep, par ^= 1) tile_body(std::true_type{}, t, it, par);
            flush_local();
        }
        for (; t < t_end; t += kStep, it += kStep, par ^= 1) tile_body(std::false_type{}, t, it, par);
        if (!kTop) {
            publish(stg_n);
            __syncwarp();
            if (lane == 0) mad_st_release_cta(&s_done[ew], 1);
        }
        if (MODE == MODE_TOP8) {
            __syncwarp();
            if (lane == 0) mad_st_release_cta(&s_done[ew], 1);
        }
        if (MODE == MODE_TOPK && row_ok) {
            const long long o = ((long long)(seg * 2 + grp) * a.M + row) * a.k;
            for (int i = 0; i < a.k; ++i) { a.topk_idx[o + i] = bi[i]; a.topk_score[o + i] = bs[i]; }
        }
    }
    tc_fence_before();
    __syncthreads();
    if (NCTA == 2) cluster_sync_all();
    if (warp == 2) {
        tc_fence_after();
        if (NCTA == 2) asm volatile("tcgen05.dealloc.cta_group::2.sync.aligned.b32 %0, %1;" ::"r"(tmem_base), "n"(TMEM_COLS) : "memory");
        else asm volatile("tcgen05.dealloc.cta_group::1.sync.aligned.b32 %0, %1;" ::"r"(tmem_base), "n"(TMEM_COLS) : "memory");
    }
}

typedef CUresult (*EncodeTiledFn)(CUtensorMap*, CUtensorMapDataType, cuuint32_t, void*, const cuuint64_t*, const cuuint64_t*,
                                  const cuuint32_t*, const cuuint32_t*, CUtensorMapInterleave, CUtensorMapSwizzle,
                                  CUtensorMapL2promotion, CUtensorMapFloatOOBfill);

EncodeTiledFn get_encode() {
    static EncodeTiledFn fn = nullptr;
    if (!fn) {
        void* p = nullptr;
        cudaDriverEntryPointQueryResult qres;
        if (cudaGetDriverEntryPoint("cuTensorMapEncodeTiled", &p, cudaEnableDefault, &qres) == cudaSuccess &&
            qres == cudaDriverEntryPointSuccess)
            fn = reinterpret_cast<EncodeTiledFn>(p);
    }
    return fn;
}

int make_map(CUtensorMap* map, const void* ptr, int rows_padded, int box_rows = BM) {
    EncodeTiledFn enc = get_encode();
    if (!enc) {
        mad_set_error("mad_match: cuTensorMapEncodeTiled is not available from the CUDA driver");
        return MAD_ERR_NODEVICE;
    }
    cuuint64_t dims[2] = {(cuuint64_t)MAD_DSC_LEN, (cuuint64_t)rows_padded};
    cuuint64_t strides[1] = {(cuuint64_t)MAD_DSC_LEN};
    cuuint32_t box[2] = {(cuuint32_t)BKB, (cuuint32_t)box_rows};
    cuuint32_t estr[2] = {1, 1};
    CUresult r = enc(map, CU_TENSOR_MAP_DATA_TYPE_UINT8, 2, const_cast<void*>(ptr), dims, strides, box, estr,
                     CU_TENSOR_MAP_INTERLEAVE_NONE, CU_TENSOR_MAP_SWIZZLE_128B, CU_TENSOR_MAP_L2_PROMOTION_L2_256B,
                     CU_TENSOR_MAP_FLOAT_OOB_FILL_NONE);
    if (r != CUDA_SUCCESS) {
        mad_set_error("mad_match: cuTensorMapEncodeTiled failed (%d)", (int)r);
        return MAD_ERR_CUDA;
    }
    return MAD_OK;
}

int check_device() {
    int dev = 0, major = 0;
    MAD_CUDA(cudaGetDevice(&dev));
    MAD_CUDA(cudaDeviceGetAttribute(&major, cudaDevAttrComputeCapabilityMajor, dev));
    if (major != 10) {
        mad_set_error("mad_match: the tcgen05 kernel needs an sm_100 device (found compute capability %d.x)", major);
        return MAD_ERR_NODEVICE;
    }
    return MAD_OK;
}

}

static int pick_ncta(int M, int N_pad);

static int u8_segments(int M, int N, double slack, int fixed_tiles) {
    if (M <= 0 || N <= 0) return 1;
    const int tn = pick_ncta(M, 256) == 2 ? 2 * BN : BN;
    const long long m_tiles = mad_ceil_div(M, BM);
    const long long n_tiles = mad_ceil_div(N, tn);
    const long long sms = mad_sm_count();
    long long best_s = 1, best_cost = -1;
    auto cost_of = [&](long long s) -> long long {
        const long long per = mad_ceil_div(n_tiles, s);
        const long long segs = mad_ceil_div(n_tiles, per);
        if (segs != s) return -1;
        return mad_ceil_div(m_tiles * s, sms) * (per + fixed_tiles);
    };
    for (long long s = 1; s <= n_tiles; ++s) {
        const long long cost = cost_of(s);
        if (cost < 0) continue;
        if (best_cost < 0 || cost < best_cost) { best_cost = cost; best_s = s; }
    }
    if (slack > 1.0)
        for (long long s = 1; s < best_s; ++s) {
            const long long cost = cost_of(s);
            if (cost >= 0 && (double)cost <= slack * (double)best_cost) return (int)s;
        }
    return (int)best_s;
}

int mad_match_u8_segments(int M, int N) { return u8_segments(M, N, 1.0, 1); }

int mad_match_u8_segments_topk(int M, int N) {
    static const int fixed = getenv("MAD_TOPK_FIXED_TILES") ? atoi(getenv("MAD_TOPK_FIXED_TILES")) : 53;
    return u8_segments(M, N, 1.0, fixed);
}

static int pick_ncta(int M, int N_pad) {
    static const bool one = getenv("MAD_MATCH_ONE_CTA") != nullptr;
    return (!one && M > BM && N_pad % 256 == 0) ? 2 : 1;
}

static int launch_common(const void* hi_u8, int M_pad, const void* lo_u8, int N_pad, int ncta, CUtensorMap* map_hi,
                         CUtensorMap* map_lo) {
    int rc = check_device();
    if (rc != MAD_OK) return rc;
    rc = make_map(map_hi, hi_u8, M_pad);
    if (rc != MAD_OK) return rc;
    (void)ncta;
    return make_map(map_lo, lo_u8, N_pad, BN);
}

template <int MODE>
static int launch_u8(int ncta, int M, int S, const CUtensorMap& map_hi, const CUtensorMap& map_lo, const U8Args& a,
                     cudaStream_t st) {
    if (ncta == 2) {
        auto kern = match_u8_kernel<MODE, 2>;
        MAD_CUDA(cudaFuncSetAttribute(kern, cudaFuncAttributeMaxDynamicSharedMemorySize, (int)SMEM_BYTES));
        cudaLaunchConfig_t cfg = {};
        cfg.gridDim = dim3(2u * (unsigned)mad_ceil_div(M, 2 * BM), (unsigned)S);
        cfg.blockDim = dim3(THREADS);
        cfg.dynamicSmemBytes = SMEM_BYTES;
        cfg.stream = st;
        cudaLaunchAttribute attr[1];
        attr[0].id = cudaLaunchAttributeClusterDimension;
        attr[0].val.clusterDim.x = 2;
        attr[0].val.clusterDim.y = 1;
        attr[0].val.clusterDim.z = 1;
        cfg.attrs = attr;
        cfg.numAttrs = 1;
        MAD_CUDA(cudaLaunchKernelEx(&cfg, kern, map_hi, map_lo, a));
    } else {
        auto kern = match_u8_kernel<MODE, 1>;
        MAD_CUDA(cudaFuncSetAttribute(kern, cudaFuncAttributeMaxDynamicSharedMemorySize, (int)SMEM_BYTES));
        dim3 grid((unsigned)mad_ceil_div(M, BM), (unsigned)S);
        kern<<<grid, THREADS, SMEM_BYTES, st>>>(map_hi, map_lo, a);
    }
    MAD_LAUNCH_OK();
    return MAD_OK;
}

int mad_match_u8_pairs(const void* hi_u8, int M, int M_pad, const void* lo_u8, int N, int N_pad, const int32_t* hi_n2,
                       const int32_t* lo_n2, const float* lo_rnorm, double cc, unsigned long long* cand_key,
                       int32_t* cand_dot, unsigned long long cap, unsigned long long* count, cudaStream_t st) {
    CUtensorMap map_hi, map_lo;
    const int ncta = pick_ncta(M, N_pad);
    int rc = launch_common(hi_u8, M_pad, lo_u8, N_pad, ncta, &map_hi, &map_lo);
    if (rc != MAD_OK) return rc;
    if (N_pad > (1 << 27)) { mad_set_error("mad_match_pairs: more than 2^27 lo rows"); return MAD_ERR_ARG; }
    U8Args a = {};
    a.M = M; a.N = N;
    a.S = mad_match_u8_segments(M, N);
    a.tiles_per_seg = (int)mad_ceil_div(mad_ceil_div(N, BN * ncta), a.S);
    a.hi_n2 = hi_n2; a.lo_n2 = lo_n2; a.lo_rnorm = lo_rnorm; a.cc = cc;
    a.cand_key = cand_key; a.cand_dot = cand_dot; a.cap = cap; a.count = count;
    a.dbg = getenv("MAD_TOPK_DBG") ? atoi(getenv("MAD_TOPK_DBG")) : 0;
    MAD_PROF("match_u8_pairs_kernel", st);
    return launch_u8<MODE_PAIRS>(ncta, M, a.S, map_hi, map_lo, a, st);
}

int mad_match_u8_topk(const void* hi_u8, int M, int M_pad, const void* lo_u8, int N, int N_pad, const int32_t* hi_n2,
                      const int32_t* lo_n2, const float* lo_rnorm, int S, int k, int lo_index_base, int32_t* topk_idx,
                      double* topk_score, cudaStream_t st) {
    CUtensorMap map_hi, map_lo;
    const int ncta = pick_ncta(M, N_pad);
    int rc = launch_common(hi_u8, M_pad, lo_u8, N_pad, ncta, &map_hi, &map_lo);
    if (rc != MAD_OK) return rc;
    U8Args a = {};
    a.M = M; a.N = N; a.S = S;
    a.tiles_per_seg = (int)mad_ceil_div(mad_ceil_div(N, BN * ncta), S);
    a.hi_n2 = hi_n2; a.lo_n2 = lo_n2; a.lo_rnorm = lo_rnorm; a.cc = 0.0;
    a.k = k; a.lo_index_base = lo_index_base; a.topk_idx = topk_idx; a.topk_score = topk_score;
    a.local_tiles = getenv("MAD_TOPK_LOCAL") ? atoi(getenv("MAD_TOPK_LOCAL")) : TOP_LOCAL_TILES;
    a.dbg = getenv("MAD_TOPK_DBG") ? atoi(getenv("MAD_TOPK_DBG")) : 0;
    if (a.dbg & 32) {
        unsigned long long z[8] = {0};
        cudaMemcpyToSymbolAsync(g_top_dbg, z, sizeof(z), 0, cudaMemcpyHostToDevice, st);
    }
    {
        MAD_PROF("match_u8_topk_kernel", st);
        rc = k <= 8 ? launch_u8<MODE_TOP8>(ncta, M, S, map_hi, map_lo, a, st) : launch_u8<MODE_TOPK>(ncta, M, S, map_hi, map_lo, a, st);
    }
    if (rc == MAD_OK && (a.dbg & 32)) {
        unsigned long long z[8];
        cudaStreamSynchronize(st);
        cudaMemcpyFromSymbol(z, g_top_dbg, sizeof(z));
        const double ctas = (double)(ncta == 2 ? 2 * mad_ceil_div(M, 2 * BM) : mad_ceil_div(M, BM)) * S;
        fprintf(stderr, "[top8 dbg] per CTA: round cycles %.0f (per epilogue warp %.0f), publish-wait cycles %.0f, publishes %.0f, rounds %.0f, "
                        "drain passes %.0f, drain busy cycles %.0f (per drain warp %.0f), inserted %.0f, stale %.0f\n",
                z[0] / ctas, z[0] / ctas / 8, z[1] / ctas, z[2] / ctas, z[3] / ctas, z[4] / ctas, z[5] / ctas, z[5] / ctas / 4, z[6] / ctas, z[7] / ctas);
    }
    return rc;
}
```

mad_b200/pipeline.py:

```python
import ctypes as C
import math
import os

import numpy as np
import torch

from . import _lib
from . import tables
from ._lib import call, KEYPOINT_DTYPE, ORIENTED_DTYPE, MAX_ORI, DSC_LEN

def launch_count():
    return int(_lib.lib.mad_launch_count())


def profile_enable(on=True):
    call("mad_profile_reset")
    call("mad_profile_enable", 1 if on else 0)


def profile_records():
    out = []
    name = C.c_char_p()
    ms = C.c_float()
    for i in range(_lib.lib.mad_profile_count()):
        call("mad_profile_get", i, C.byref(name), C.byref(ms))
        out.append((name.value.decode(), float(ms.value)))
    call("mad_profile_reset")
    return out


def _require_cuda():
    if not torch.cuda.is_available():
        raise _lib.MadError("mad_b200 needs a CUDA device (sm_100a); there is no CPU fallback")


def _stream():
    return C.c_void_p(torch.cuda.current_stream().cuda_stream)


def _ptr(t):
    return C.c_void_p(t.data_ptr()) if t is not None else C.c_void_p(0)


class _Readback(object):
    _slots = {}

    @classmethod
    def read(cls, *tensors):
        dev = tensors[0].device
        key = (dev.index, torch.cuda.current_stream().cuda_stream)
        slot = cls._slots.get(key)
        if slot is None:
            slot = cls._slots[key] = torch.zeros(512, dtype=torch.int64).pin_memory()
        st = _stream()
        off, views = 0, []
        for t in tensors:
            t = t.contiguous().view(-1)
            nbytes = t.numel() * t.element_size()
            assert nbytes % 4 == 0 and off + nbytes <= slot.numel() * 8
            call("mad_publish_small", _ptr(t), C.c_void_p(slot.data_ptr() + off), nbytes, st)
            views.append((off, t.dtype, t.numel()))
            off += (nbytes + 7) // 8 * 8
        torch.cuda.current_stream().synchronize()
        raw = slot.numpy()
        out = []
        for o, dt, n in views:
            a = raw.view(np.uint8)[o:o + n * (8 if dt == torch.int64 else 4)].view(np.int64 if dt == torch.int64 else np.int32)
            out.extend(int(v) for v in a)
        return out


def _dptr(a):
    return a.ctypes.data_as(C.c_void_p)


class _DeviceTables(object):

    def __init__(self, device, ori_zones=112, dsc_zones=16):
        self.device = device
        self.keep = []
        self.z_ori = self._zone_struct(tables.zone_tables(ori_zones))
        self.z_dsc = self._zone_struct(tables.zone_tables(dsc_zones))
        ot = tables.orientation_tables(ori_zones)
        self.ori_zones = ori_zones
        self.r1 = torch.from_numpy(np.ascontiguousarray(ot.r1.reshape(-1, 9))).to(device)
        self.rf = torch.from_numpy(np.ascontiguousarray(ot.rf.reshape(-1, 9))).to(device)
        self.rf_inv = torch.from_numpy(np.ascontiguousarray(ot.rf_inv.reshape(-1, 9))).to(device)

    def _zone_struct(self, zt):
        b = torch.from_numpy(np.ascontiguousarray(zt.bounds)).to(self.device)
        f = torch.from_numpy(np.ascontiguousarray(zt.belt_first)).to(self.device)
        p = torch.from_numpy(np.ascontiguousarray(zt.belt_phi)).to(self.device)
        self.keep += [b, f, p]
        s = _lib.MadZoneTable()
        s.n_zones, s.n_belts = zt.size, zt.n_belts
        s.bounds, s.belt_first, s.belt_phi = b.data_ptr(), f.data_ptr(), p.data_ptr()
        s.fast = None
        fast = torch.zeros(_lib.ZONE_FAST_BYTES, dtype=torch.uint8, device=self.device)
        with torch.cuda.device(self.device):
            call("mad_zone_fast_build", C.byref(s), _ptr(fast), _stream())
            torch.cuda.current_stream().synchronize()
        self.keep.append(fast)
        s.fast = fast.data_ptr()
        return s


_TABLE_CACHE = {}


def device_tables(device):
    key = (str(device),)
    if key not in _TABLE_CACHE:
        _TABLE_CACHE[key] = _DeviceTables(device)
    return _TABLE_CACHE[key]


class Space(object):

    def __init__(self):
        self.grids = []
        self.logs = []
        self.gauss = []
        self.grad4 = []
        self.grad_flags = []
        self.dims = []
        self.n_oct = 2
        self.n_input_voxels = 0
        self._gauss = []
        self._grad_done = {}

    @property
    def dims_host(self):
        return np.array([d for o in self.dims for d in o], dtype=np.int32)


def gradient_reach(radius):
    up = max(2 * radius, int(math.ceil((2 * radius - 1) * math.sqrt(3.0))) + 1)
    base = max(radius, int(math.ceil((radius - 0.5) * math.sqrt(3.0))) + 1)
    return up, base


def ensure_gradient(space, kp, radius=8):
    if all(f is None for f in space.grad_flags[:space.n_oct]) or len(kp) == 0:
        return
    key = (id(kp), int(radius))
    if key in space._grad_done:
        return
    st = _stream()
    up, base = gradient_reach(int(radius))
    f0, f1 = space.grad_flags
    if f0 is None or f1 is None:
        raise _lib.MadError("ensure_gradient: octaves must share the gradient mode")
    call("mad_gradient_mark", _ptr(kp.table), len(kp), _dptr(space.dims_host), up, base, _ptr(f0), _ptr(f1), st)
    for o, (gx, gy, gz) in enumerate(space.dims[:space.n_oct]):
        call("mad_gradient_masked", _ptr(space._gauss[o]), gx, gy, gz, _ptr(space.grad4[o]), _ptr(space.grad_flags[o]), st)
    space._grad_done[key] = kp


def full_gradient(space):
    st = _stream()
    for o, (gx, gy, gz) in enumerate(space.dims[:space.n_oct]):
        fl = space.grad_flags[o]
        if fl is None:
            continue
        fl[fl == 0] = 1
        call("mad_gradient_masked", _ptr(space._gauss[o]), gx, gy, gz, _ptr(space.grad4[o]), _ptr(fl), st)
        space.grad_flags[o] = None
    space.grad_flags = [None] * len(space.grad_flags)
    return space.grad4


def build_space(grid, map_padding=9, sig_init=2, sig_presmooth=1, exact_f64=True, keep_gauss=True, full_gradient=True,
                oct_mode="both"):
    _require_cuda()
    if isinstance(grid, np.ndarray):
        grid = torch.from_numpy(np.ascontiguousarray(grid, dtype=np.float32)).cuda()
    grid = grid.contiguous().float()
    dev = grid.device
    st = _stream()
    nx, ny, nz = grid.shape
    sp = Space()
    sp.n_input_voxels = nx * ny * nz
    if map_padding:
        bx, by, bz = nx + 2 * map_padding, ny + 2 * map_padding, nz + 2 * map_padding
        base = torch.empty((bx, by, bz), dtype=torch.float32, device=dev)
        call("mad_pad3d", _ptr(grid), nx, ny, nz, int(map_padding), _ptr(base), st)
    else:
        bx, by, bz = nx, ny, nz
        base = grid
    if oct_mode not in ("both", "up", "base"):
        raise _lib.MadError("build_space: oct_mode %r" % (oct_mode,))
    ux, uy, uz = 2 * bx - 1, 2 * by - 1, 2 * bz - 1
    if oct_mode != "base":
        up = torch.empty((ux, uy, uz), dtype=torch.float32, device=dev)
        ws_bytes = _lib.lib.mad_upsample_workspace_bytes(bx, by, bz)
        ws = torch.empty(ws_bytes, dtype=torch.uint8, device=dev)
        if sig_presmooth:
            rad = tables.gaussian_radius(sig_presmooth)
            gw = np.ascontiguousarray(tables.gaussian_weights(sig_presmooth, 0, rad))
            call("mad_upsample_presmooth", _ptr(base), bx, by, bz, _dptr(gw), rad, _ptr(up), _ptr(ws), ws_bytes, st)
        else:
            call("mad_upsample_presmooth", _ptr(base), bx, by, bz, C.c_void_p(0), 0, _ptr(up), _ptr(ws), ws_bytes, st)
        del ws
    if oct_mode == "both":
        sp.grids = [up, base]
        sp.dims = [(ux, uy, uz), (bx, by, bz)]
    else:
        sp.n_oct = 1
        sp.grids = [up] if oct_mode == "up" else [base]
        sp.dims = [(ux, uy, uz) if oct_mode == "up" else (bx, by, bz)]
    rad = tables.gaussian_radius(sig_init)
    w0 = np.ascontiguousarray(tables.gaussian_weights(sig_init, 0, rad))
    w2 = np.ascontiguousarray(tables.gaussian_weights(sig_init, 2, rad))
    scale = float(np.float32(sig_init ** 2))
    for g, (gx, gy, gz) in zip(sp.grids, sp.dims):
        ws_bytes = _lib.lib.mad_log_gauss_workspace_bytes(gx, gy, gz)
        ws = torch.empty(ws_bytes, dtype=torch.uint8, device=dev)
        lg = torch.empty((gx, gy, gz), dtype=torch.float32, device=dev)
        gs = torch.empty((gx, gy, gz), dtype=torch.float32, device=dev)
        call("mad_log_gauss", _ptr(g), gx, gy, gz, _dptr(w0), _dptr(w2), rad, C.c_float(scale), _ptr(lg), _ptr(gs),
             _ptr(ws), ws_bytes, 1 if exact_f64 else 0, st)
        del ws
        gr = torch.empty((gx, gy, gz, 4), dtype=torch.float32, device=dev)
        if full_gradient:
            call("mad_gradient", _ptr(gs), gx, gy, gz, _ptr(gr), st)
            sp.grad_flags.append(None)
        else:
            sp.grad_flags.append(torch.zeros(_lib.lib.mad_gradient_tiles(gx, gy, gz), dtype=torch.uint8, device=dev))
        sp._gauss.append(gs)
        sp.logs.append(lg)
        sp.gauss.append(gs if keep_gauss else None)
        sp.grad4.append(gr)
    if full_gradient and not keep_gauss:
        sp._gauss = []
    if sp.n_oct == 1:
        sp.dims.append((1, 1, 1))
        sp.grad4.append(torch.zeros((1, 1, 1, 4), dtype=torch.float32, device=dev))
        sp.grad_flags.append(None if full_gradient else torch.zeros(1, dtype=torch.uint8, device=dev))
    return sp


class Keypoints(object):

    def __init__(self, table, count):
        self.table = table
        self.count = int(count)
        self._host = None

    def host(self):
        if self._host is None:
            self._host = self.table[:self.count].cpu().numpy().view(KEYPOINT_DTYPE).reshape(-1)
        return self._host

    def __len__(self):
        return self.count


def keypoints_from_host(arr, device):
    arr = np.ascontiguousarray(arr, dtype=KEYPOINT_DTYPE)
    t = torch.from_numpy(arr.view(np.int32).reshape(-1, 12).copy()).to(device)
    k = Keypoints(t, len(arr))
    k._host = arr
    return k


def detect(space, border=12, threshold=5e-2, cap=None):
    _require_cuda()
    dev = space.logs[0].device
    st = _stream()
    if cap is None:
        cap = 1 << 16
    while True:
        cand = torch.empty((cap, 12), dtype=torch.int32, device=dev)
        counter = torch.zeros(1, dtype=torch.int32, device=dev)
        for o, (lg, (gx, gy, gz)) in enumerate(zip(space.logs, space.dims)):
            call("mad_detect", _ptr(lg), gx, gy, gz, o, int(border), C.c_float(threshold), _ptr(cand), cap,
                 _ptr(counter), st)
        n = _Readback.read(counter)[0]
        if n <= cap:
            break
        cap = int(n * 1.25) + 16
    out = torch.empty((max(n, 1), 12), dtype=torch.int32, device=dev)
    out_count = torch.zeros(1, dtype=torch.int32, device=dev)
    ws_bytes = _lib.lib.mad_sort_keypoints_workspace_bytes(n)
    ws = torch.empty(max(ws_bytes, 1), dtype=torch.uint8, device=dev)
    dims = space.dims_host
    call("mad_sort_keypoints", _ptr(cand), n, _dptr(dims), _ptr(out), _ptr(out_count), _ptr(ws), ws_bytes, st)
    return Keypoints(out, _Readback.read(out_count)[0])


class Oriented(object):
    def __init__(self, table, count):
        self.table = table
        self.count = int(count)
        self._host = None

    def host(self):
        if self._host is None:
            self._host = self.table[:self.count].cpu().numpy().view(ORIENTED_DTYPE).reshape(-1)
        return self._host

    def __len__(self):
        return self.count


def oriented_from_host(arr, device):
    arr = np.ascontiguousarray(arr, dtype=ORIENTED_DTYPE)
    t = torch.from_numpy(arr.view(np.int32).reshape(-1, 2).copy()).to(device)
    o = Oriented(t, len(arr))
    o._host = arr
    return o


def orient(space, kp, radius=8, lim_main=6, lim_sec=6):
    _require_cuda()
    dev = space.grad4[0].device
    st = _stream()
    tb = device_tables(dev)
    n = len(kp)
    if n == 0:
        return Oriented(torch.empty((1, 2), dtype=torch.int32, device=dev), 0)
    ensure_gradient(space, kp, radius)
    n_ori = torch.empty(n, dtype=torch.int32, device=dev)
    slots = torch.empty((n, MAX_ORI), dtype=torch.int32, device=dev)
    dims = space.dims_host
    call("mad_orient", _ptr(space.grad4[0]), _ptr(space.grad4[1]), _dptr(dims), _ptr(kp.table), n, int(radius),
         C.byref(tb.z_ori), _ptr(tb.r1), int(lim_main), int(lim_sec), _ptr(n_ori), _ptr(slots), st)
    cap = n * MAX_ORI
    out = torch.empty((cap, 2), dtype=torch.int32, device=dev)
    out_count = torch.zeros(1, dtype=torch.int32, device=dev)
    ws_bytes = _lib.lib.mad_compact_oriented_workspace_bytes(n)
    ws = torch.empty(ws_bytes, dtype=torch.uint8, device=dev)
    call("mad_compact_oriented", _ptr(n_ori), _ptr(slots), n, _ptr(out), cap, _ptr(out_count), _ptr(ws), ws_bytes, st)
    return Oriented(out, _Readback.read(out_count)[0])


def describe(space, kp, ori, radius=8):
    _require_cuda()
    dev = space.grad4[0].device
    st = _stream()
    tb = device_tables(dev)
    d = len(ori)
    dsc = torch.empty((d, DSC_LEN), dtype=torch.int16, device=dev)
    if d == 0:
        return dsc
    ensure_gradient(space, kp, radius)
    dims = space.dims_host
    call("mad_describe", _ptr(space.grad4[0]), _ptr(space.grad4[1]), _dptr(dims), _ptr(kp.table), _ptr(ori.table), d,
         int(radius), C.byref(tb.z_dsc), _ptr(tb.rf), _ptr(tb.rf_inv), tb.ori_zones, _ptr(dsc), st)
    return dsc


def describe_struct(grid, patch_size=16, map_padding=9, sig_init=2, sig_presmooth=1, exact_f64=True,
                    keep_gauss=False, full_gradient=None):
    r = (patch_size - patch_size % 2) // 2
    if full_gradient is None:
        full_gradient = bool(keep_gauss)
    sp = build_space(grid, map_padding, sig_init, sig_presmooth, exact_f64=exact_f64, keep_gauss=keep_gauss,
                     full_gradient=full_gradient)
    kp = detect(sp)
    ori = orient(sp, kp, r)
    dsc = describe(sp, kp, ori, r)
    return sp, kp, ori, dsc


class DescriptorSet(object):

    def __init__(self, dsc, need_half=False):
        _require_cuda()
        if isinstance(dsc, np.ndarray):
            dsc = torch.from_numpy(np.ascontiguousarray(dsc, dtype=np.int16)).cuda()
        self.dsc = dsc.contiguous()
        assert self.dsc.dtype == torch.int16 and self.dsc.dim() == 2 and self.dsc.shape[1] == DSC_LEN
        dev = self.dsc.device
        st = _stream()
        self.rows = self.dsc.shape[0]
        self.rows_padded = max((self.rows + 255) // 256 * 256, 256)
        self.norm2 = torch.empty(max(self.rows, 1), dtype=torch.int32, device=dev)
        self.rnorm = torch.empty(self.rows_padded, dtype=torch.float32, device=dev)
        self.u8 = torch.empty((self.rows_padded, DSC_LEN), dtype=torch.uint8, device=dev)
        mx = torch.zeros(2, dtype=torch.int32, device=dev)
        call("mad_dsc_prepare", _ptr(self.dsc), self.rows, self.rows_padded, _ptr(self.norm2), _ptr(self.rnorm),
             _ptr(self.u8), _ptr(mx), _ptr(mx[1:]), st)
        self._max_dev = mx
        self._max_entry = None
        self._max_norm2 = None
        self.half = None
        s = _lib.MadDscSet()
        s.dsc = self.dsc.data_ptr()
        s.half = 0
        s.norm2 = self.norm2.data_ptr()
        s.u8 = self.u8.data_ptr()
        s.rnorm = self.rnorm.data_ptr()
        s.rows, s.rows_padded = self.rows, self.rows_padded
        s.max_entry = -1
        s.max_norm2 = -1
        self.c = s
        if need_half:
            self.ensure_half()

    @property
    def max_entry(self):
        if self._max_entry is None:
            self._set_maxima(*self._max_dev.tolist())
        return self._max_entry

    def _set_maxima(self, max_entry, max_norm2):
        self._max_entry, self._max_norm2 = int(max_entry), int(max_norm2)
        self.c.max_entry, self.c.max_norm2 = self._max_entry, self._max_norm2

    def ensure_half(self):
        if self.half is None:
            self.half = torch.empty((self.rows_padded, DSC_LEN), dtype=torch.float16, device=self.dsc.device)
            call("mad_dsc_to_half", _ptr(self.dsc), self.rows, self.rows_padded, _ptr(self.half), _stream())
            self.c.half = self.half.data_ptr()
        return self


def _as_set(x):
    return x if isinstance(x, DescriptorSet) else DescriptorSet(x)


def _check_descriptors(hi, lo):
    if max(hi._max_entry, lo._max_entry) >= _lib.DSC_REFUSED:
        raise _lib.MadError("mad_match: not a descriptor set (a negative entry, or a squared norm >= 2^31)")


def _exact_impl(hi, lo):
    _check_descriptors(hi, lo)
    if max(hi._max_entry, lo._max_entry) <= 255:
        return 0
    if max(hi._max_entry, lo._max_entry) <= 2048 and hi._max_norm2 * lo._max_norm2 <= 1 << 48:
        return 2
    return 1


def _pick_impl(hi, lo, impl):
    verify = False
    if impl is None:
        if hi._max_entry is None or lo._max_entry is None:
            return 0, True
        impl = _exact_impl(hi, lo)
    return _pick_impl_explicit(hi, lo, impl), verify


def _pick_impl_explicit(hi, lo, impl):
    hi.max_entry, lo.max_entry
    if impl == 2:
        hi.ensure_half()
        lo.ensure_half()
    return impl


_PAIR_CAP = {}


def scores_from_dots(pair_hi, pair_lo, pair_dot, hi_norm2, lo_norm2):
    p = np.asarray(hi_norm2, dtype=np.float64)[np.asarray(pair_hi)] * np.asarray(lo_norm2, dtype=np.float64)[np.asarray(pair_lo)]
    out = np.zeros(len(p), dtype=np.float64)
    nz = p > 0.0
    out[nz] = np.asarray(pair_dot, dtype=np.float64)[nz] / np.sqrt(p[nz])
    return out


def pair_hi_from_counts(counts):
    counts = np.asarray(counts)
    return np.repeat(np.arange(len(counts), dtype=np.int32), counts)


def match_threshold(hi, lo, cc=0.6, impl=None, want="score"):
    hi, lo = _as_set(hi), _as_set(lo)
    dev = hi.dsc.device
    st = _stream()
    m = hi.rows
    if m == 0 or lo.rows == 0:
        e = torch.empty(0, dtype=torch.int32, device=dev)
        return e, e.clone(), torch.empty(0, dtype=torch.float64, device=dev)
    impl, verify = _pick_impl(hi, lo, impl)
    if impl == 0:
        return _match_threshold_onepass(hi, lo, cc, dev, st, verify, want)
    if want != "score":
        raise _lib.MadError("match_threshold: want='dot' is a format of the uint8 kernel (impl 0)")
    n_seg = int(_lib.lib.mad_match_segments(m, lo.rows, impl))
    seg_count = torch.empty(m * n_seg, dtype=torch.int32, device=dev)
    call("mad_match_count", C.byref(hi.c), C.byref(lo.c), C.c_double(cc), n_seg, _ptr(seg_count), impl, st)
    seg_off = torch.empty(m * n_seg, dtype=torch.int64, device=dev)
    total = torch.zeros(1, dtype=torch.int64, device=dev)
    ws_bytes = _lib.lib.mad_exclusive_scan_workspace_bytes(m * n_seg)
    ws = torch.empty(ws_bytes, dtype=torch.uint8, device=dev)
    call("mad_exclusive_scan_i32_to_i64", _ptr(seg_count), m * n_seg, _ptr(seg_off), _ptr(total), _ptr(ws), ws_bytes, st)
    p = int(total.item())
    pair_hi = torch.empty(max(p, 1), dtype=torch.int32, device=dev)
    pair_lo = torch.empty(max(p, 1), dtype=torch.int32, device=dev)
    score = torch.empty(max(p, 1), dtype=torch.float64, device=dev)
    call("mad_match_fill", C.byref(hi.c), C.byref(lo.c), C.c_double(cc), n_seg, _ptr(seg_off), _ptr(pair_hi), _ptr(pair_lo),
         _ptr(score), impl, st)
    return pair_hi[:p], pair_lo[:p], score[:p]


def _read_counts(count, hi, lo):
    vals = _Readback.read(count, hi._max_dev, lo._max_dev)
    hi._set_maxima(vals[1], vals[2])
    lo._set_maxima(vals[3], vals[4])
    return int(vals[0])


def _match_threshold_onepass(hi, lo, cc, dev, st, verify=False, want="score"):
    key = (hi.rows, lo.rows)
    cap = _PAIR_CAP.get(key, max(1 << 20, 16 * (hi.rows + lo.rows)))
    while True:
        cand_key = torch.empty(cap, dtype=torch.int64, device=dev)
        cand_dot = torch.empty(cap, dtype=torch.int32, device=dev)
        count = torch.empty(1, dtype=torch.int64, device=dev)
        call("mad_match_pairs", C.byref(hi.c), C.byref(lo.c), C.c_double(cc), _ptr(cand_key), _ptr(cand_dot),
             C.c_uint64(cap), _ptr(count), st)
        p = _read_counts(count, hi, lo)
        if p >= (1 << 62):
            raise _lib.MadError("mad_match_pairs: the kernel's internal hand-off timed out (pair list incomplete)")
        if verify and _exact_impl(hi, lo) != 0:
            if want != "score":
                raise _lib.MadError("match_threshold: entries above 255 need the fp16 or SIMT kernel, which have no want='dot' form")
            return match_threshold(hi, lo, cc)
        if p <= cap:
            break
        cap = p + p // 8 + 1024
    _PAIR_CAP[key] = max(cap, p + p // 4)
    pair_hi = torch.empty(max(p, 1), dtype=torch.int32, device=dev)
    pair_lo = torch.empty(max(p, 1), dtype=torch.int32, device=dev)
    score = torch.empty(max(p, 1), dtype=torch.float64 if want == "score" else torch.int32, device=dev)
    if p:
        ws_bytes = _lib.lib.mad_match_pairs_finish_workspace_bytes(p)
        ws = torch.empty(ws_bytes, dtype=torch.uint8, device=dev)
        if want == "score":
            call("mad_match_pairs_finish", _ptr(cand_key), _ptr(cand_dot), p, hi.rows, lo.rows, _ptr(hi.norm2), _ptr(lo.norm2),
                 _ptr(pair_hi), _ptr(pair_lo), _ptr(score), _ptr(ws), ws_bytes, st)
        else:
            call("mad_match_pairs_finish_dot", _ptr(cand_key), _ptr(cand_dot), p, hi.rows, lo.rows, _ptr(pair_hi), _ptr(pair_lo),
                 _ptr(score), _ptr(ws), ws_bytes, st)
    return pair_hi[:p], pair_lo[:p], score[:p]


HOST_COPY_CTAS = int(os.environ.get("MAD_HOST_COPY_CTAS", "8"))


class HostStage(object):

    def __init__(self):
        self.bufs = {}
        self.copy_stream = None
        self.keep = []

    def fetch(self, name, t, overlap=False):
        n = t.numel() * t.element_size()
        buf = self.bufs.get(name)
        if buf is None or buf.numel() < n:
            if buf is not None:
                self.keep.append(buf)
            buf = torch.empty(max(n * 5 // 4, 256), dtype=torch.uint8).pin_memory()
            self.bufs[name] = buf
        view = buf[:n].view(t.dtype).view(t.shape)
        if not n:
            return view
        if overlap:
            if self.copy_stream is None:
                self.copy_stream = torch.cuda.Stream()
            self.copy_stream.wait_stream(torch.cuda.current_stream())
            t = t.contiguous()
            if t.data_ptr() % 16 == 0:
                call("mad_copy_to_host", _ptr(t), C.c_void_p(buf.data_ptr()), n, HOST_COPY_CTAS, C.c_void_p(self.copy_stream.cuda_stream))
            else:
                with torch.cuda.stream(self.copy_stream):
                    view.copy_(t, non_blocking=True)
            t.record_stream(self.copy_stream)
            self.keep.append(t)
        else:
            view.copy_(t, non_blocking=True)
        return view

    def sync(self):
        torch.cuda.current_stream().synchronize()
        if self.copy_stream is not None:
            self.copy_stream.synchronize()
        self.keep = []
        self.marks = []

    def mark(self):
        evs = [torch.cuda.Event()]
        evs[0].record(torch.cuda.current_stream())
        if self.copy_stream is not None:
            evs.append(torch.cuda.Event())
            evs[1].record(self.copy_stream)
        self.marks = evs

    def wait(self):
        for ev in getattr(self, "marks", []):
            ev.synchronize()
        self.marks = []
        self.keep = []


class MapStream(object):

    def __init__(self, hi=None, cc=0.6, exact_f64=True, match_impl=None, patch_size=16, depth=2, download=True, compact=False):
        _require_cuda()
        self.compact = bool(compact)
        self.download = download
        self.hi = _as_set(hi) if hi is not None else None
        self.cc, self.exact, self.impl, self.patch = cc, exact_f64, match_impl, patch_size
        self.up_stream = torch.cuda.Stream()
        self.stages = [HostStage() for _ in range(max(2, depth))]
        self.n = 0
        self.gbuf = [None] * max(2, depth)
        self.gfree = [None] * max(2, depth)
        self.n_up = 0

    def upload(self, grid):
        if isinstance(grid, np.ndarray):
            grid = torch.from_numpy(np.ascontiguousarray(grid, dtype=np.float32))
        if self.n_up - self.n >= len(self.gbuf):
            raise _lib.MadError("MapStream.upload: %d uploads are waiting for submit(); the %d upload buffers are all in use"
                                % (self.n_up - self.n, len(self.gbuf)))
        k = self.n_up % len(self.gbuf)
        self.n_up += 1
        dev = torch.device("cuda", torch.cuda.current_device())
        if self.gbuf[k] is None or self.gbuf[k].shape != grid.shape:
            self.gbuf[k] = torch.empty(tuple(grid.shape), dtype=torch.float32, device=dev)
        if self.gfree[k] is not None:
            self.up_stream.wait_event(self.gfree[k])
        with torch.cuda.stream(self.up_stream):
            self.gbuf[k].copy_(grid, non_blocking=True)
            ev = torch.cuda.Event()
            ev.record(self.up_stream)
        return self.gbuf[k], ev, k

    def submit(self, uploaded):
        g, ev, k = uploaded
        cur = torch.cuda.current_stream()
        cur.wait_event(ev)
        stage = self.stages[self.n % len(self.stages)]
        self.n += 1
        stage.wait()
        sp, kp, ori, dsc = describe_struct(g, patch_size=self.patch, exact_f64=self.exact)
        if k is not None:
            self.gfree[k] = torch.cuda.Event()
            self.gfree[k].record(cur)
        get = (lambda name, t: stage.fetch(name, t, overlap=True)) if self.download else (lambda name, t: t)
        out = {"kp": get("kp", kp.table[:len(kp)]), "ori": get("ori", ori.table[:len(ori)])}
        lo = DescriptorSet(dsc) if (self.hi is not None or self.compact) else None
        if self.compact:
            out.update(dsc_u8=get("dsc8", lo.u8[:lo.rows]), lo_norm2=get("n2", lo.norm2[:lo.rows]))
        else:
            out["dsc"] = get("dsc", dsc)
        if self.hi is not None:
            if self.compact:
                ph, pl, dot = match_threshold(self.hi, lo, self.cc, impl=self.impl, want="dot")
                cnt = torch.zeros(self.hi.rows, dtype=torch.int32, device=ph.device)
                if ph.numel():
                    cnt.scatter_add_(0, ph.long(), torch.ones_like(ph))
                out.update(pair_hi_counts=get("pc", cnt), pair_lo=get("pl", pl), pair_dot=get("pd", dot))
            else:
                ph, pl, sc = match_threshold(self.hi, lo, self.cc, impl=self.impl)
                out.update(pair_hi=get("ph", ph), pair_lo=get("pl", pl), score=get("sc", sc))
        stage.mark()
        return stage, out

    def result(self, ticket):
        stage, out = ticket
        stage.wait()
        return out


class MapBatch(object):

    def __init__(self, streams=4, patch_size=16, exact_f64=True, compact=False):
        _require_cuda()
        from concurrent.futures import ThreadPoolExecutor
        self.compact = bool(compact)
        self.nw = max(1, int(streams))
        self.patch, self.exact = patch_size, exact_f64
        self.device = torch.cuda.current_device()
        self.streams = [torch.cuda.Stream() for _ in range(self.nw)]
        self.stages = [HostStage() for _ in range(self.nw)]
        self.up = [None] * self.nw
        self.pool = ThreadPoolExecutor(self.nw)
        self.last_d2h_bytes = 0
        device_tables(torch.device("cuda", self.device))

    def _work(self, w, grids, download):
        torch.cuda.set_device(self.device)
        out = []
        with torch.cuda.stream(self.streams[w]):
            for j in range(w, len(grids), self.nw):
                g = grids[j]
                if isinstance(g, np.ndarray):
                    g = torch.from_numpy(np.ascontiguousarray(g, dtype=np.float32))
                if not g.is_cuda:
                    if self.up[w] is None or self.up[w].shape != g.shape:
                        self.up[w] = torch.empty(tuple(g.shape), dtype=torch.float32, device="cuda")
                    self.up[w].copy_(g, non_blocking=True)
                    g = self.up[w]
                sp, kp, ori, dsc = describe_struct(g, patch_size=self.patch, exact_f64=self.exact)
                r = {"n_kp": len(kp), "n_dsc": len(ori)}
                if download:
                    st = self.stages[w]
                    r.update(kp=st.fetch("kp%d" % j, kp.table[:len(kp)]), ori=st.fetch("ori%d" % j, ori.table[:len(ori)]))
                    if self.compact:
                        ds = DescriptorSet(dsc)
                        r["_max"] = ds._max_dev[:1]
                        r["dsc_u8"] = st.fetch("dsc8_%d" % j, ds.u8[:ds.rows])
                        r["_dsc_dev"] = dsc
                    else:
                        r["dsc"] = st.fetch("dsc%d" % j, dsc)
                else:
                    r.update(dsc=dsc, kp=kp.table[:len(kp)], ori=ori.table[:len(ori)])
                out.append((j, r))
            self.streams[w].synchronize()
            for _, r in out:
                if "_max" in r:
                    if int(r.pop("_max").item()) > 255:
                        del r["dsc_u8"]
                        r["dsc"] = r["_dsc_dev"].cpu()
                    del r["_dsc_dev"]
        return out

    def run(self, grids, download=True):
        main = torch.cuda.current_stream()
        for s_ in self.streams:
            s_.wait_stream(main)
        parts = [f.result() for f in [self.pool.submit(self._work, w, grids, download) for w in range(self.nw)]]
        for s_ in self.streams:
            main.wait_stream(s_)
        res = [r for _, r in sorted((x for p in parts for x in p), key=lambda x: x[0])]
        if download:
            self.last_d2h_bytes = int(sum(r[k].numel() * r[k].element_size() for r in res for k in ("dsc", "dsc_u8", "kp", "ori") if k in r))
        return res


def concat_sets(sets):
    offs = np.cumsum([0] + [s.rows for s in sets]).astype(np.int64)
    return DescriptorSet(torch.cat([s.dsc for s in sets], 0)), offs


def match_topk(hi, lo, k=8, lo_index_base=0, impl=None):
    hi, lo = _as_set(hi), _as_set(lo)
    dev = hi.dsc.device
    st = _stream()
    impl, verify = _pick_impl(hi, lo, impl)
    idx = torch.empty((hi.rows, k), dtype=torch.int32, device=dev)
    score = torch.empty((hi.rows, k), dtype=torch.float64, device=dev)
    ws_bytes = _lib.lib.mad_match_topk_workspace_bytes(hi.rows, lo.rows, int(k), impl)
    ws = torch.empty(ws_bytes, dtype=torch.uint8, device=dev)
    call("mad_match_topk", C.byref(hi.c), C.byref(lo.c), int(k), int(lo_index_base), _ptr(idx), _ptr(score), _ptr(ws),
         ws_bytes, impl, st)
    if verify:
        _read_counts(torch.zeros(1, dtype=torch.int64, device=dev), hi, lo)
        if _exact_impl(hi, lo) != 0:
            return match_topk(hi, lo, k, lo_index_base)
    return idx, score


def topk_merge(idx_g, score_g):
    g, m, k = idx_g.shape
    dev = idx_g.device
    idx = torch.empty((m, k), dtype=torch.int32, device=dev)
    score = torch.empty((m, k), dtype=torch.float64, device=dev)
    call("mad_topk_merge", _ptr(idx_g.contiguous()), _ptr(score_g.contiguous()), g, m, k, _ptr(idx), _ptr(score), _stream())
    return idx, score


class FeatureTable(object):

    def __init__(self, dsc, index, oct_scale, main_bin, sec_bin, subv_map_coords):
        _require_cuda()
        self.set = dsc if isinstance(dsc, DescriptorSet) else DescriptorSet(dsc)
        dev = self.set.dsc.device
        meta = np.stack([np.asarray(index), np.asarray(oct_scale), np.asarray(main_bin), np.asarray(sec_bin)], 1)
        self.meta_host = np.ascontiguousarray(meta, dtype=np.int32)
        self.subv_host = np.ascontiguousarray(subv_map_coords, dtype=np.float64).reshape(-1, 3)
        assert len(self.meta_host) == self.set.rows == len(self.subv_host)
        self.meta = torch.from_numpy(self.meta_host).to(dev)
        self.subv = torch.from_numpy(self.subv_host).to(dev)

    @classmethod
    def from_features(cls, df_list):
        dsc = np.array([df.lin_ar_subeqsp for df in df_list], dtype=np.int16).reshape(-1, DSC_LEN)
        return cls(dsc, [df.index for df in df_list], [df.oct_scale for df in df_list], [df.main_bin for df in df_list],
                   [df.sec_bin for df in df_list], np.array([df.subv_map_coords for df in df_list], dtype=np.float64))


def _cloud_grid(cloud, cell):
    org = cloud.min(0) - cell
    dims = (np.floor((cloud.max(0) - org) / cell).astype(np.int64) + 2)
    cidx = np.floor((cloud - org) / cell).astype(np.int64)
    lin = (cidx[:, 0] * dims[1] + cidx[:, 1]) * dims[2] + cidx[:, 2]
    order = np.argsort(lin, kind="stable")
    ncell = int(dims.prod())
    cell_start = np.zeros(ncell + 1, dtype=np.int32)
    np.cumsum(np.bincount(lin, minlength=ncell), out=cell_start[1:])
    occ = np.zeros(tuple(dims), dtype=bool)
    occ[cidx[:, 0], cidx[:, 1], cidx[:, 2]] = True
    near = np.zeros_like(occ)
    p = np.pad(occ, 1)
    for dx in range(3):
        for dy in range(3):
            for dz in range(3):
                near |= p[dx:dx + dims[0], dy:dy + dims[1], dz:dz + dims[2]]
    bits = np.packbits(near.reshape(-1), bitorder="little")
    bits = np.concatenate([bits, np.zeros((-len(bits)) % 4, dtype=np.uint8)]).view(np.uint32)
    return np.ascontiguousarray(cloud[order]), cell_start, bits, org.astype(np.float64), dims.astype(np.int32)


def match_dsc(lo, hi, anchor_dist_thresh=4, cc_threshold=0.65, impl=None):
    dev = hi.set.dsc.device
    st = _stream()
    ph, pl, sc = match_threshold(hi.set, lo.set, cc_threshold, impl=impl)
    p = int(ph.numel())
    if p == 0:
        return torch.empty((0, 23), dtype=torch.float64, device=dev), np.zeros((0, 3)), np.zeros((0, 3))
    used_hi = torch.zeros(hi.set.rows, dtype=torch.uint8, device=dev)
    used_lo = torch.zeros(lo.set.rows, dtype=torch.uint8, device=dev)
    call("mad_mark_used", _ptr(ph), p, _ptr(used_hi), st)
    call("mad_mark_used", _ptr(pl), p, _ptr(used_lo), st)
    hi_cloud = np.unique(hi.subv_host[used_hi.cpu().numpy().astype(bool)], axis=0)
    lo_cloud = np.unique(lo.subv_host[used_lo.cpu().numpy().astype(bool)], axis=0)
    lo_sorted, cell_start, bits, org, dims = _cloud_grid(lo_cloud, float(anchor_dist_thresh))
    tb = device_tables(dev)
    d_hi_cloud = torch.from_numpy(np.ascontiguousarray(hi_cloud)).to(dev)
    d_lo_sorted = torch.from_numpy(lo_sorted).to(dev)
    d_cell_start = torch.from_numpy(cell_start).to(dev)
    d_bits = torch.from_numpy(bits.view(np.int32)).to(dev)
    results = torch.empty((p, 23), dtype=torch.float64, device=dev)
    call("mad_repeatability", _ptr(ph), _ptr(pl), _ptr(sc), p, _ptr(hi.subv), _ptr(lo.subv), _ptr(hi.meta), _ptr(lo.meta),
         _ptr(tb.rf), _ptr(tb.rf_inv), tb.ori_zones, _ptr(d_hi_cloud), len(hi_cloud), _ptr(d_lo_sorted), _ptr(d_cell_start),
         _ptr(d_bits), _dptr(org), _dptr(dims), C.c_double(float(anchor_dist_thresh)), _ptr(results), st)
    return results, lo_cloud, hi_cloud


def match_dsc_lists(lo_dsc_list, hi_dsc_list, anchor_dist_thresh=4, cc_threshold=0.65):
    res, lo_cloud, hi_cloud = match_dsc(FeatureTable.from_features(lo_dsc_list), FeatureTable.from_features(hi_dsc_list),
                                        anchor_dist_thresh, cc_threshold)
    return list(res.cpu().numpy()), lo_cloud, hi_cloud
```

Measured before the change: 2.242 billion.

## Replace pair radix sort with bucket counting and in-bucket ranking

The match kernel now counts accepted pairs into (row, column-bucket) histograms as it emits candidates. A scan, a scatter into buckets and an in-bucket rank kernel then produce the ordered pair list, replacing the full 64-bit CUB radix sort and its finish kernel. The place step is launched before the host waits on the count readback, so host sync overlaps GPU work. Cached maxima are no longer re-read. dsc_prepare gets coalesced loads and stores plus per-block atomics. This costs atomics in the hot match kernel and quadratic in-bucket ranking, and output buffers are sized to the cap.

Result: faster. 2.294 billion (median of 6 runs) (+2.3%).

```diff
diff --git a/include/mad_b200.h b/include/mad_b200.h
--- a/include/mad_b200.h
+++ b/include/mad_b200.h
@@ -134,15 +134,12 @@
 int mad_exclusive_scan_i32_to_i64(const int32_t* in, int n, int64_t* out, int64_t* total,
                                   void* workspace, size_t workspace_bytes, void* stream);
 
-int mad_match_pairs(const MadDscSet* hi, const MadDscSet* lo, double cc, uint64_t* cand_key, int32_t* cand_dot,
-                    uint64_t cap, uint64_t* count, void* stream);
-size_t mad_match_pairs_finish_workspace_bytes(long long n);
-int mad_match_pairs_finish(const uint64_t* cand_key, const int32_t* cand_dot, long long n, int hi_rows, int lo_rows,
-                           const int32_t* hi_n2, const int32_t* lo_n2, int32_t* pair_hi, int32_t* pair_lo,
-                           double* pair_score, void* workspace, size_t workspace_bytes, void* stream);
-int mad_match_pairs_finish_dot(const uint64_t* cand_key, const int32_t* cand_dot, long long n, int hi_rows, int lo_rows,
-                               int32_t* pair_hi, int32_t* pair_lo, int32_t* pair_dot, void* workspace, size_t workspace_bytes,
-                               void* stream);
+size_t mad_match_pairs_workspace_bytes(int hi_rows, int lo_rows, uint64_t cap);
+int mad_match_pairs_find(const MadDscSet* hi, const MadDscSet* lo, double cc, uint64_t cap, uint64_t* count, void* workspace,
+                         size_t workspace_bytes, void* stream);
+int mad_match_pairs_place(const MadDscSet* hi, const MadDscSet* lo, uint64_t cap, const uint64_t* count, int32_t* pair_hi,
+                          int32_t* pair_lo, double* pair_score, int32_t* pair_dot, void* workspace, size_t workspace_bytes,
+                          void* stream);
 
 size_t mad_match_topk_workspace_bytes(int M, int N, int k, int impl);
 int mad_match_topk(const MadDscSet* hi, const MadDscSet* lo, int k, int lo_index_base,
diff --git a/mad_b200/_lib.py b/mad_b200/_lib.py
--- a/mad_b200/_lib.py
+++ b/mad_b200/_lib.py
@@ -79,10 +79,9 @@
     "mad_compact_oriented": (_I, [_P, _P, _I, _P, _I, _P, _P, _SZ, _P]),
     "mad_describe": (_I, [_P, _P, _P, _P, _P, _I, _I, C.POINTER(MadZoneTable), _P, _P, _I, _P, _P]),
     "mad_dsc_prepare": (_I, [_P, _I, _I, _P, _P, _P, _P, _P, _P]),
-    "mad_match_pairs": (_I, [C.POINTER(MadDscSet), C.POINTER(MadDscSet), C.c_double, _P, _P, C.c_uint64, _P, _P]),
-    "mad_match_pairs_finish_workspace_bytes": (_SZ, [C.c_longlong]),
-    "mad_match_pairs_finish": (_I, [_P, _P, C.c_longlong, _I, _I, _P, _P, _P, _P, _P, _P, _SZ, _P]),
-    "mad_match_pairs_finish_dot": (_I, [_P, _P, C.c_longlong, _I, _I, _P, _P, _P, _P, _SZ, _P]),
+    "mad_match_pairs_workspace_bytes": (_SZ, [_I, _I, C.c_uint64]),
+    "mad_match_pairs_find": (_I, [C.POINTER(MadDscSet), C.POINTER(MadDscSet), C.c_double, C.c_uint64, _P, _P, _SZ, _P]),
+    "mad_match_pairs_place": (_I, [C.POINTER(MadDscSet), C.POINTER(MadDscSet), C.c_uint64, _P, _P, _P, _P, _P, _P, _SZ, _P]),
     "mad_dsc_norms": (_I, [_P, _I, _P, _P]),
     "mad_dsc_to_half": (_I, [_P, _I, _I, _P, _P]),
     "mad_match_segments": (_I, [_I, _I, _I]),
diff --git a/mad_b200/csrc/api.cu b/mad_b200/csrc/api.cu
--- a/mad_b200/csrc/api.cu
+++ b/mad_b200/csrc/api.cu
@@ -157,8 +157,8 @@
 extern "C" int mad_match_count(const MadDscSet* hi, const MadDscSet* lo, double cc, int n_seg, int32_t* seg_count,
                                int impl, void* stream) {
     if (impl == 0) {
-        mad_set_error("%s: impl 0 (the one-pass uint8 tcgen05 kernel) has no count/fill form -- call mad_match_pairs + "
-                      "mad_match_pairs_finish; count/fill serve impl 1 (SIMT check) and 2 (fp16 tcgen05)", "mad_match_count");
+        mad_set_error("%s: impl 0 (the one-pass uint8 tcgen05 kernel) has no count/fill form -- call "
+                      "mad_match_pairs_find + mad_match_pairs_place; count/fill serve impl 1 (SIMT check) and 2 (fp16 tcgen05)", "mad_match_count");
         return MAD_ERR_ARG;
     }
     int rc = check_sets(hi, lo, impl);
@@ -178,8 +178,8 @@
 extern "C" int mad_match_fill(const MadDscSet* hi, const MadDscSet* lo, double cc, int n_seg, const int64_t* seg_offset,
                               int32_t* pair_hi, int32_t* pair_lo, double* pair_score, int impl, void* stream) {
     if (impl == 0) {
-        mad_set_error("%s: impl 0 (the one-pass uint8 tcgen05 kernel) has no count/fill form -- call mad_match_pairs + "
-                      "mad_match_pairs_finish; count/fill serve impl 1 (SIMT check) and 2 (fp16 tcgen05)", "mad_match_fill");
+        mad_set_error("%s: impl 0 (the one-pass uint8 tcgen05 kernel) has no count/fill form -- call "
+                      "mad_match_pairs_find + mad_match_pairs_place; count/fill serve impl 1 (SIMT check) and 2 (fp16 tcgen05)", "mad_match_fill");
         return MAD_ERR_ARG;
     }
     int rc = check_sets(hi, lo, impl);
diff --git a/mad_b200/csrc/match_common.cuh b/mad_b200/csrc/match_common.cuh
--- a/mad_b200/csrc/match_common.cuh
+++ b/mad_b200/csrc/match_common.cuh
@@ -126,7 +126,8 @@
 int mad_match_u8_segments_topk(int M, int N);
 int mad_match_u8_pairs(const void* hi_u8, int M, int M_pad, const void* lo_u8, int N, int N_pad, const int32_t* hi_n2,
                        const int32_t* lo_n2, const float* lo_rnorm, double cc, unsigned long long* cand_key,
-                       int32_t* cand_dot, unsigned long long cap, unsigned long long* count, cudaStream_t st);
+                       int32_t* cand_dot, unsigned long long cap, unsigned long long* count, int32_t* bkt_count, int bkt_n,
+                       int bkt_shift, cudaStream_t st);
 int mad_match_u8_topk(const void* hi_u8, int M, int M_pad, const void* lo_u8, int N, int N_pad, const int32_t* hi_n2,
                       const int32_t* lo_n2, const float* lo_rnorm, int S, int k, int lo_index_base, int32_t* topk_idx,
                       double* topk_score, cudaStream_t st);
diff --git a/mad_b200/csrc/match_prep.cu b/mad_b200/csrc/match_prep.cu
--- a/mad_b200/csrc/match_prep.cu
+++ b/mad_b200/csrc/match_prep.cu
@@ -1,4 +1,6 @@
 #include <cub/cub.cuh>
+
+#include <algorithm>
 
 #include "common.cuh"
 #include "match_common.cuh"
@@ -9,38 +11,39 @@
 dsc_prepare_kernel(const int16_t* __restrict__ dsc, int rows, int rows_padded, int32_t* __restrict__ norm2,
                    float* __restrict__ rnorm, uint8_t* __restrict__ u8, int32_t* __restrict__ max_entry,
                    int32_t* __restrict__ max_norm2) {
+    __shared__ int s_mx[8], s_n2[8];
     const int row = (int)((blockIdx.x * (long long)blockDim.x + threadIdx.x) >> 5);
-    const int lane = threadIdx.x & 31;
-    if (row >= rows_padded) return;
+    const int lane = threadIdx.x & 31, w = threadIdx.x >> 5;
+    const bool active = row < rows_padded;
     long long acc = 0;
     int mx = 0;
-    uint32_t packed[8];
-    if (row < rows) {
-        const uint4* src = reinterpret_cast<const uint4*>(dsc + (long long)row * MAD_DSC_LEN + lane * 32);
+    uint2 packed[4];
+    if (active && row < rows) {
+        const uint4* src = reinterpret_cast<const uint4*>(dsc + (long long)row * MAD_DSC_LEN);
 #pragma unroll
         for (int q = 0; q < 4; ++q) {
-            const uint4 v = __ldg(src + q);
-            const uint32_t w[4] = {v.x, v.y, v.z, v.w};
+            const uint4 v = __ldg(src + q * 32 + lane);
+            const uint32_t wd[4] = {v.x, v.y, v.z, v.w};
+            uint32_t pk[2] = {0u, 0u};
 #pragma unroll
             for (int h = 0; h < 4; ++h) {
-                const int e0 = (int)(int16_t)(w[h] & 0xFFFFu), e1 = (int)(int16_t)(w[h] >> 16);
+                const int e0 = (int)(int16_t)(wd[h] & 0xFFFFu), e1 = (int)(int16_t)(wd[h] >> 16);
                 acc += (long long)e0 * e0 + (long long)e1 * e1;
                 mx = max(mx, max(e0, e1));
                 if (e0 < 0 || e1 < 0) mx = MAD_DSC_REFUSED;
                 const uint32_t b0 = (uint32_t)min(max(e0, 0), 255), b1 = (uint32_t)min(max(e1, 0), 255);
-                const int slot = q * 8 + h * 2;
-                if ((slot & 3) == 0) packed[slot >> 2] = b0 | (b1 << 8);
-                else packed[slot >> 2] |= (b0 << 16) | (b1 << 24);
+                pk[h >> 1] |= (b0 | (b1 << 8)) << (16 * (h & 1));
             }
+            packed[q] = make_uint2(pk[0], pk[1]);
         }
     } else {
 #pragma unroll
-        for (int q = 0; q < 8; ++q) packed[q] = 0;
-    }
-    if (u8) {
-        uint4* dst = reinterpret_cast<uint4*>(u8 + (long long)row * MAD_DSC_LEN + lane * 32);
-        dst[0] = make_uint4(packed[0], packed[1], packed[2], packed[3]);
-        dst[1] = make_uint4(packed[4], packed[5], packed[6], packed[7]);
+        for (int q = 0; q < 4; ++q) packed[q] = make_uint2(0u, 0u);
+    }
+    if (active && u8) {
+        uint2* dst = reinterpret_cast<uint2*>(u8 + (long long)row * MAD_DSC_LEN);
+#pragma unroll
+        for (int q = 0; q < 4; ++q) dst[q * 32 + lane] = packed[q];
     }
 #pragma unroll
     for (int o = 16; o > 0; o >>= 1) {
@@ -49,56 +52,100 @@
     }
     if (lane == 0) {
         if (acc > 0x7FFFFFFFLL) mx = MAD_DSC_REFUSED;
-        if (row < rows) norm2[row] = (int32_t)acc;
-        rnorm[row] = acc > 0 ? (float)(1.0 / sqrt((double)acc)) : 0.f;
-        if (mx > 0) atomicMax(max_entry, mx);
-        if (max_norm2 && acc > 0) atomicMax(max_norm2, (int32_t)min(acc, 0x7FFFFFFFLL));
-    }
-}
-
-__global__ void pairs_finish_kernel(const unsigned long long* __restrict__ key, const int32_t* __restrict__ dot,
-                                    long long n, unsigned long long lo_rows, const int32_t* __restrict__ hi_n2,
-                                    const int32_t* __restrict__ lo_n2,
-                                    int32_t* __restrict__ pair_hi, int32_t* __restrict__ pair_lo,
-                                    double* __restrict__ score) {
+        if (active) {
+            if (row < rows) norm2[row] = (int32_t)acc;
+            rnorm[row] = acc > 0 ? (float)(1.0 / sqrt((double)acc)) : 0.f;
+        }
+        s_mx[w] = mx;
+        s_n2[w] = (int)min(acc, 0x7FFFFFFFLL);
+    }
+    __syncthreads();
+    if (threadIdx.x == 0) {
+        int m = 0, n = 0;
+        for (int i = 0; i < (int)(blockDim.x >> 5); ++i) { m = max(m, s_mx[i]); n = max(n, s_n2[i]); }
+        if (m > 0) atomicMax(max_entry, m);
+        if (max_norm2 && n > 0) atomicMax(max_norm2, n);
+    }
+}
+
+struct BucketShape {
+    int n, shift;
+    long long total;
+};
+
+BucketShape bucket_shape(int hi_rows, int lo_rows) {
+    BucketShape b;
+    b.shift = 5;
+    while (b.shift < 31 && (long long)hi_rows * (((long long)lo_rows + (1LL << b.shift) - 1) >> b.shift) > (1LL << 23)) ++b.shift;
+    b.n = (int)(((long long)lo_rows + (1LL << b.shift) - 1) >> b.shift);
+    b.total = (long long)hi_rows * b.n;
+    return b;
+}
+
+struct OrderedLayout {
+    size_t key_off, dot_off, cnt_off, off_off, row_off, col_off, bdot_off, scan_off, scan_bytes, total;
+};
+
+OrderedLayout ordered_layout(int hi_rows, int lo_rows, unsigned long long cap) {
+    OrderedLayout L;
+    const size_t c = cap > 0 ? (size_t)cap : 1;
+    const size_t nb1 = (size_t)bucket_shape(hi_rows, lo_rows).total + 1;
+    L.key_off = 0;
+    L.dot_off = mad_align_up(c * sizeof(unsigned long long), 256);
+    L.cnt_off = L.dot_off + mad_align_up(c * sizeof(int32_t), 256);
+    L.off_off = L.cnt_off + mad_align_up(nb1 * sizeof(int32_t), 256);
+    L.row_off = L.off_off + mad_align_up(nb1 * sizeof(int32_t), 256);
+    L.col_off = L.row_off + mad_align_up(c * sizeof(int32_t), 256);
+    L.bdot_off = L.col_off + mad_align_up(c * sizeof(int32_t), 256);
+    L.scan_off = L.bdot_off + mad_align_up(c * sizeof(int32_t), 256);
+    size_t b = 0;
+    cub::DeviceScan::ExclusiveSum(nullptr, b, (const int32_t*)nullptr, (int32_t*)nullptr, (int)nb1);
+    L.scan_bytes = mad_align_up(b, 256);
+    L.total = L.scan_off + L.scan_bytes;
+    return L;
+}
+
+__global__ void pairs_zero_kernel(unsigned long long* count, int4* cnt, long long n4) {
+    const long long i0 = blockIdx.x * (long long)blockDim.x + threadIdx.x;
+    if (i0 == 0) *count = 0ull;
+    for (long long i = i0; i < n4; i += (long long)gridDim.x * blockDim.x) cnt[i] = make_int4(0, 0, 0, 0);
+}
+
+__global__ void pairs_bucket_kernel(const unsigned long long* __restrict__ key, const int32_t* __restrict__ dot,
+                                    const unsigned long long* __restrict__ count, unsigned long long cap,
+                                    int bn, int shift, int32_t* __restrict__ cnt,
+                                    const int32_t* __restrict__ off, int32_t* __restrict__ brow, int32_t* __restrict__ bcol,
+                                    int32_t* __restrict__ bdot) {
+    const unsigned long long n = *count;
     const long long i = blockIdx.x * (long long)blockDim.x + threadIdx.x;
-    if (i >= n) return;
+    if (n > cap || (unsigned long long)i >= n) return;
     const unsigned long long k = key[i];
-    const int row = (int)(k / lo_rows), col = (int)(k % lo_rows);
-    pair_hi[i] = row;
-    pair_lo[i] = col;
-    score[i] = mad_score(dot[i], (double)__ldg(hi_n2 + row), (double)__ldg(lo_n2 + col));
-}
-
-__global__ void pairs_finish_dot_kernel(const unsigned long long* __restrict__ key, const int32_t* __restrict__ dot, long long n,
-                                        unsigned long long lo_rows, int32_t* __restrict__ pair_hi, int32_t* __restrict__ pair_lo,
-                                        int32_t* __restrict__ pair_dot) {
+    const int row = (int)(k >> 32), col = (int)(k & 0xFFFFFFFFull);
+    const long long b = (long long)row * bn + (col >> shift);
+    const int slot = off[b] + atomicSub(cnt + b, 1) - 1;
+    brow[slot] = row;
+    bcol[slot] = col;
+    bdot[slot] = dot[i];
+}
+
+__global__ void pairs_order_kernel(const int32_t* __restrict__ brow, const int32_t* __restrict__ bcol,
+                                   const int32_t* __restrict__ bdot, const unsigned long long* __restrict__ count,
+                                   unsigned long long cap, const int32_t* __restrict__ off, int bn, int shift,
+                                   const int32_t* __restrict__ hi_n2, const int32_t* __restrict__ lo_n2,
+                                   int32_t* __restrict__ pair_hi, int32_t* __restrict__ pair_lo, double* __restrict__ score,
+                                   int32_t* __restrict__ pair_dot) {
+    const unsigned long long n = *count;
     const long long i = blockIdx.x * (long long)blockDim.x + threadIdx.x;
-    if (i >= n) return;
-    const unsigned long long k = key[i];
-    pair_hi[i] = (int)(k / lo_rows);
-    pair_lo[i] = (int)(k % lo_rows);
-    pair_dot[i] = dot[i];
-}
-
-__global__ void zero_u64_kernel(unsigned long long* p) { *p = 0ull; }
-
-struct FinishLayout {
-    size_t key_off, dot_off, cub_off, cub_bytes, total;
-};
-
-FinishLayout finish_layout(long long n) {
-    FinishLayout L;
-    const size_t nn = (size_t)(n > 0 ? n : 1);
-    L.key_off = 0;
-    L.dot_off = mad_align_up(nn * sizeof(unsigned long long), 256);
-    L.cub_off = L.dot_off + mad_align_up(nn * sizeof(int32_t), 256);
-    size_t b = 0;
-    cub::DeviceRadixSort::SortPairs(nullptr, b, (const unsigned long long*)nullptr, (unsigned long long*)nullptr,
-                                    (const int32_t*)nullptr, (int32_t*)nullptr, (int)nn, 0, 64);
-    L.cub_bytes = mad_align_up(b, 256);
-    L.total = L.cub_off + L.cub_bytes;
-    return L;
+    if (n > cap || (unsigned long long)i >= n) return;
+    const int row = brow[i], col = bcol[i];
+    const long long b = (long long)row * bn + (col >> shift);
+    const int b0 = off[b], b1 = off[b + 1];
+    int pos = b0;
+    for (int j = b0; j < b1; ++j) pos += bcol[j] < col ? 1 : 0;
+    pair_hi[pos] = row;
+    pair_lo[pos] = col;
+    if (score) score[pos] = mad_score(bdot[i], (double)__ldg(hi_n2 + row), (double)__ldg(lo_n2 + col));
+    else pair_dot[pos] = bdot[i];
 }
 
 }
@@ -116,83 +163,95 @@
     return MAD_OK;
 }
 
-extern "C" int mad_match_pairs(const MadDscSet* hi, const MadDscSet* lo, double cc, uint64_t* cand_key, int32_t* cand_dot,
-                               uint64_t cap, uint64_t* count, void* stream) {
-    MAD_CHECK_ARG(hi && lo && count && hi->rows >= 0 && lo->rows >= 0);
-    cudaStream_t st = (cudaStream_t)stream;
-    {
-        MAD_PROF("zero_u64_kernel", st);
-        zero_u64_kernel<<<1, 1, 0, st>>>(reinterpret_cast<unsigned long long*>(count));
-        MAD_LAUNCH_OK();
-    }
-    if (hi->rows == 0 || lo->rows == 0) return MAD_OK;
+static int pairs_launch(const MadDscSet* hi, const MadDscSet* lo, double cc, uint64_t* cand_key, int32_t* cand_dot,
+                        uint64_t cap, uint64_t* count, int32_t* bkt_count, int bkt_n, int bkt_shift, cudaStream_t st) {
     MAD_CHECK_ARG(hi->u8 && lo->u8 && hi->norm2 && lo->norm2 && lo->rnorm && cand_key && cand_dot);
     MAD_CHECK_ARG(hi->rows_padded >= hi->rows && hi->rows_padded % 128 == 0);
     MAD_CHECK_ARG(lo->rows_padded >= lo->rows && lo->rows_padded % 128 == 0);
-    int rc = mad_check_descriptor_sets(hi, lo, "mad_match_pairs");
+    int rc = mad_check_descriptor_sets(hi, lo, "mad_match_pairs_find");
     if (rc != MAD_OK) return rc;
     if (hi->max_entry > 255 || lo->max_entry > 255) {
-        mad_set_error("mad_match_pairs: descriptor entries up to %d do not fit the uint8 tensor-core operand "
+        mad_set_error("mad_match_pairs_find: descriptor entries up to %d do not fit the uint8 tensor-core operand "
                       "(use mad_match_count/mad_match_fill with impl = 2 or 1)",
                       hi->max_entry > lo->max_entry ? hi->max_entry : lo->max_entry);
         return MAD_ERR_ARG;
     }
     return mad_match_u8_pairs(hi->u8, hi->rows, hi->rows_padded, lo->u8, lo->rows, lo->rows_padded, hi->norm2, lo->norm2,
                               lo->rnorm, cc, reinterpret_cast<unsigned long long*>(cand_key), cand_dot,
-                              (unsigned long long)cap, reinterpret_cast<unsigned long long*>(count), st);
-}
-
-extern "C" size_t mad_match_pairs_finish_workspace_bytes(long long n) { return finish_layout(n).total; }
-
-static int pairs_finish_impl(const uint64_t* cand_key, const int32_t* cand_dot, long long n, int hi_rows, int lo_rows,
-                             const int32_t* hi_n2, const int32_t* lo_n2, int32_t* pair_hi, int32_t* pair_lo, double* pair_score,
-                             int32_t* pair_dot, void* workspace, size_t workspace_bytes, void* stream);
-
-extern "C" int mad_match_pairs_finish(const uint64_t* cand_key, const int32_t* cand_dot, long long n, int hi_rows,
-                                      int lo_rows, const int32_t* hi_n2, const int32_t* lo_n2, int32_t* pair_hi, int32_t* pair_lo,
-                                      double* pair_score, void* workspace, size_t workspace_bytes, void* stream) {
-    MAD_CHECK_ARG(n >= 0 && n < (1LL << 31));
-    if (n == 0) return MAD_OK;
-    MAD_CHECK_ARG(hi_n2 && lo_n2 && pair_score);
-    return pairs_finish_impl(cand_key, cand_dot, n, hi_rows, lo_rows, hi_n2, lo_n2, pair_hi, pair_lo, pair_score, nullptr, workspace,
-                             workspace_bytes, stream);
-}
-
-extern "C" int mad_match_pairs_finish_dot(const uint64_t* cand_key, const int32_t* cand_dot, long long n, int hi_rows, int lo_rows,
-                                          int32_t* pair_hi, int32_t* pair_lo, int32_t* pair_dot, void* workspace,
-                                          size_t workspace_bytes, void* stream) {
-    MAD_CHECK_ARG(n >= 0 && n < (1LL << 31));
-    if (n == 0) return MAD_OK;
-    MAD_CHECK_ARG(pair_dot);
-    return pairs_finish_impl(cand_key, cand_dot, n, hi_rows, lo_rows, nullptr, nullptr, pair_hi, pair_lo, nullptr, pair_dot, workspace,
-                             workspace_bytes, stream);
-}
-
-static int pairs_finish_impl(const uint64_t* cand_key, const int32_t* cand_dot, long long n, int hi_rows, int lo_rows,
-                             const int32_t* hi_n2, const int32_t* lo_n2, int32_t* pair_hi, int32_t* pair_lo, double* pair_score,
-                             int32_t* pair_dot, void* workspace, size_t workspace_bytes, void* stream) {
-    MAD_CHECK_ARG(cand_key && cand_dot && pair_hi && pair_lo && workspace && hi_rows > 0 && lo_rows > 0);
-    const FinishLayout L = finish_layout(n);
+                              (unsigned long long)cap, reinterpret_cast<unsigned long long*>(count), bkt_count, bkt_n, bkt_shift, st);
+}
+
+extern "C" size_t mad_match_pairs_workspace_bytes(int hi_rows, int lo_rows, uint64_t cap) {
+    return ordered_layout(hi_rows > 0 ? hi_rows : 0, lo_rows > 0 ? lo_rows : 0, cap).total;
+}
+
+struct OrderedBuffers {
+    unsigned long long *key, *count;
+    int32_t *dot, *cnt, *off, *brow, *bcol, *bdot;
+    char* scan;
+};
+
+static OrderedBuffers ordered_buffers(const OrderedLayout& L, void* workspace, uint64_t* count) {
+    char* ws = reinterpret_cast<char*>(workspace);
+    OrderedBuffers b;
+    b.key = reinterpret_cast<unsigned long long*>(ws + L.key_off);
+    b.count = reinterpret_cast<unsigned long long*>(count);
+    b.dot = reinterpret_cast<int32_t*>(ws + L.dot_off);
+    b.cnt = reinterpret_cast<int32_t*>(ws + L.cnt_off);
+    b.off = reinterpret_cast<int32_t*>(ws + L.off_off);
+    b.brow = reinterpret_cast<int32_t*>(ws + L.row_off);
+    b.bcol = reinterpret_cast<int32_t*>(ws + L.col_off);
+    b.bdot = reinterpret_cast<int32_t*>(ws + L.bdot_off);
+    b.scan = ws + L.scan_off;
+    return b;
+}
+
+extern "C" int mad_match_pairs_find(const MadDscSet* hi, const MadDscSet* lo, double cc, uint64_t cap, uint64_t* count,
+                                    void* workspace, size_t workspace_bytes, void* stream) {
+    MAD_CHECK_ARG(hi && lo && count && workspace && hi->rows >= 0 && lo->rows >= 0 && cap < (1ull << 31));
+    cudaStream_t st = (cudaStream_t)stream;
+    const OrderedLayout L = ordered_layout(hi->rows, lo->rows, cap);
     MAD_CHECK_ARG(workspace_bytes >= L.total);
+    const BucketShape B = bucket_shape(hi->rows, lo->rows);
+    const OrderedBuffers W = ordered_buffers(L, workspace, count);
+    const long long n4 = mad_ceil_div(B.total + 1, 4);
+    {
+        MAD_PROF("pairs_zero_kernel", st);
+        pairs_zero_kernel<<<(unsigned)std::min<long long>(std::max<long long>(mad_ceil_div(n4, 256), 1), 4096), 256, 0, st>>>(
+            W.count, reinterpret_cast<int4*>(W.cnt), n4);
+        MAD_LAUNCH_OK();
+    }
+    if (hi->rows == 0 || lo->rows == 0) return MAD_OK;
+    int rc = pairs_launch(hi, lo, cc, reinterpret_cast<uint64_t*>(W.key), W.dot, cap, count, W.cnt, B.n, B.shift, st);
+    if (rc != MAD_OK) return rc;
+    MAD_PROF("pairs_bucket_scan", st);
+    size_t b = L.scan_bytes;
+    MAD_CUDA(cub::DeviceScan::ExclusiveSum(W.scan, b, W.cnt, W.off, (int)(B.total + 1), st));
+    return MAD_OK;
+}
+
+extern "C" int mad_match_pairs_place(const MadDscSet* hi, const MadDscSet* lo, uint64_t cap, const uint64_t* count,
+                                     int32_t* pair_hi, int32_t* pair_lo, double* pair_score, int32_t* pair_dot, void* workspace,
+                                     size_t workspace_bytes, void* stream) {
+    MAD_CHECK_ARG(hi && lo && count && workspace && hi->rows >= 0 && lo->rows >= 0 && cap < (1ull << 31));
+    MAD_CHECK_ARG(pair_hi && pair_lo && (pair_score == nullptr) != (pair_dot == nullptr));
+    if (hi->rows == 0 || lo->rows == 0) return MAD_OK;
+    MAD_CHECK_ARG(hi->norm2 && lo->norm2);
     cudaStream_t st = (cudaStream_t)stream;
-    char* ws = reinterpret_cast<char*>(workspace);
-    unsigned long long* key_sorted = reinterpret_cast<unsigned long long*>(ws + L.key_off);
-    int32_t* dot_sorted = reinterpret_cast<int32_t*>(ws + L.dot_off);
-    int key_bits = 1;
-    while (key_bits < 64 && (1ULL << key_bits) < (unsigned long long)hi_rows * (unsigned long long)lo_rows) ++key_bits;
-    size_t b = L.cub_bytes;
+    const OrderedLayout L = ordered_layout(hi->rows, lo->rows, cap);
+    MAD_CHECK_ARG(workspace_bytes >= L.total);
+    const BucketShape B = bucket_shape(hi->rows, lo->rows);
+    const OrderedBuffers W = ordered_buffers(L, workspace, const_cast<uint64_t*>(count));
+    const unsigned grid = (unsigned)std::max<long long>(mad_ceil_div((long long)cap, 256), 1);
     {
-        MAD_PROF("cub_radix_sort_pairs", st);
-        MAD_CUDA(cub::DeviceRadixSort::SortPairs(ws + L.cub_off, b, reinterpret_cast<const unsigned long long*>(cand_key),
-                                                 key_sorted, cand_dot, dot_sorted, (int)n, 0, key_bits, st));
-    }
-    MAD_PROF("pairs_finish_kernel", st);
-    if (pair_dot)
-        pairs_finish_dot_kernel<<<(unsigned)mad_ceil_div(n, 256), 256, 0, st>>>(key_sorted, dot_sorted, n, (unsigned long long)lo_rows, pair_hi,
-                                                                               pair_lo, pair_dot);
-    else
-        pairs_finish_kernel<<<(unsigned)mad_ceil_div(n, 256), 256, 0, st>>>(key_sorted, dot_sorted, n, (unsigned long long)lo_rows, hi_n2, lo_n2,
-                                                                           pair_hi, pair_lo, pair_score);
+        MAD_PROF("pairs_bucket_kernel", st);
+        pairs_bucket_kernel<<<grid, 256, 0, st>>>(W.key, W.dot, W.count, cap, B.n, B.shift, W.cnt, W.off,
+                                                  W.brow, W.bcol, W.bdot);
+        MAD_LAUNCH_OK();
+    }
+    MAD_PROF("pairs_order_kernel", st);
+    pairs_order_kernel<<<grid, 256, 0, st>>>(W.brow, W.bcol, W.bdot, W.count, cap, W.off, B.n, B.shift, hi->norm2, lo->norm2, pair_hi,
+                                             pair_lo, pair_score, pair_dot);
     MAD_LAUNCH_OK();
     return MAD_OK;
 }
diff --git a/mad_b200/csrc/match_u8.cu b/mad_b200/csrc/match_u8.cu
--- a/mad_b200/csrc/match_u8.cu
+++ b/mad_b200/csrc/match_u8.cu
@@ -147,6 +147,8 @@
     int32_t* cand_dot;
     unsigned long long cap;
     unsigned long long* count;
+    int32_t* bkt_count;
+    int bkt_n, bkt_shift;
     int k, lo_index_base;
     int local_tiles;
     int dbg;
@@ -322,7 +324,8 @@
                             if (p > 0.0 && a.cc > 0.0 && lhs > rhs * (1.0 + 1e-13)) ok[k] = true;
                             else if (p > 0.0 && a.cc > 0.0 && lhs < rhs * (1.0 - 1e-13)) ok[k] = false;
                             else ok[k] = mad_score(dot[k], n2r, n2c) > a.cc;
-                            ent[k] = (unsigned long long)row * (unsigned long long)a.N + (unsigned long long)(low >> 5);
+                            ent[k] = ((unsigned long long)row << 32) | (unsigned long long)(low >> 5);
+                            if (ok[k]) atomicAdd(a.bkt_count + (long long)row * a.bkt_n + (int)((low >> 5) >> a.bkt_shift), 1);
                         }
                         const unsigned m = __ballot_sync(0xFFFFFFFFu, ok[k]);
                         pos[k] = total + __popc(m & ((1u << lane) - 1u));
@@ -798,18 +801,20 @@
 
 int mad_match_u8_pairs(const void* hi_u8, int M, int M_pad, const void* lo_u8, int N, int N_pad, const int32_t* hi_n2,
                        const int32_t* lo_n2, const float* lo_rnorm, double cc, unsigned long long* cand_key,
-                       int32_t* cand_dot, unsigned long long cap, unsigned long long* count, cudaStream_t st) {
+                       int32_t* cand_dot, unsigned long long cap, unsigned long long* count, int32_t* bkt_count, int bkt_n,
+                       int bkt_shift, cudaStream_t st) {
     CUtensorMap map_hi, map_lo;
     const int ncta = pick_ncta(M, N_pad);
     int rc = launch_common(hi_u8, M_pad, lo_u8, N_pad, ncta, &map_hi, &map_lo);
     if (rc != MAD_OK) return rc;
-    if (N_pad > (1 << 27)) { mad_set_error("mad_match_pairs: more than 2^27 lo rows"); return MAD_ERR_ARG; }
+    if (N_pad > (1 << 27)) { mad_set_error("mad_match_pairs_find: more than 2^27 lo rows"); return MAD_ERR_ARG; }
     U8Args a = {};
     a.M = M; a.N = N;
     a.S = mad_match_u8_segments(M, N);
     a.tiles_per_seg = (int)mad_ceil_div(mad_ceil_div(N, BN * ncta), a.S);
     a.hi_n2 = hi_n2; a.lo_n2 = lo_n2; a.lo_rnorm = lo_rnorm; a.cc = cc;
     a.cand_key = cand_key; a.cand_dot = cand_dot; a.cap = cap; a.count = count;
+    a.bkt_count = bkt_count; a.bkt_n = bkt_n; a.bkt_shift = bkt_shift;
     a.dbg = getenv("MAD_TOPK_DBG") ? atoi(getenv("MAD_TOPK_DBG")) : 0;
     MAD_PROF("match_u8_pairs_kernel", st);
     return launch_u8<MODE_PAIRS>(ncta, M, a.S, map_hi, map_lo, a, st);
diff --git a/mad_b200/pipeline.py b/mad_b200/pipeline.py
--- a/mad_b200/pipeline.py
+++ b/mad_b200/pipeline.py
@@ -46,7 +46,7 @@
     _slots = {}
 
     @classmethod
-    def read(cls, *tensors):
+    def read(cls, *tensors, then=None):
         dev = tensors[0].device
         key = (dev.index, torch.cuda.current_stream().cuda_stream)
         slot = cls._slots.get(key)
@@ -61,7 +61,13 @@
             call("mad_publish_small", _ptr(t), C.c_void_p(slot.data_ptr() + off), nbytes, st)
             views.append((off, t.dtype, t.numel()))
             off += (nbytes + 7) // 8 * 8
-        torch.cuda.current_stream().synchronize()
+        if then is None:
+            torch.cuda.current_stream().synchronize()
+        else:
+            ev = torch.cuda.Event()
+            ev.record()
+            then()
+            ev.synchronize()
         raw = slot.numpy()
         out = []
         for o, dt, n in views:
@@ -498,10 +504,11 @@
     return pair_hi[:p], pair_lo[:p], score[:p]
 
 
-def _read_counts(count, hi, lo):
-    vals = _Readback.read(count, hi._max_dev, lo._max_dev)
-    hi._set_maxima(vals[1], vals[2])
-    lo._set_maxima(vals[3], vals[4])
+def _read_counts(count, hi, lo, then=None):
+    sets = [s for s in (hi, lo) if s._max_entry is None]
+    vals = _Readback.read(count, *[s._max_dev for s in sets], then=then)
+    for i, s in enumerate(sets):
+        s._set_maxima(vals[1 + 2 * i], vals[2 + 2 * i])
     return int(vals[0])
 
 
@@ -509,14 +516,22 @@
     key = (hi.rows, lo.rows)
     cap = _PAIR_CAP.get(key, max(1 << 20, 16 * (hi.rows + lo.rows)))
     while True:
-        cand_key = torch.empty(cap, dtype=torch.int64, device=dev)
-        cand_dot = torch.empty(cap, dtype=torch.int32, device=dev)
+        if cap >= (1 << 31):
+            raise _lib.MadError("match_threshold: more than 2^31 - 1 pairs")
+        pair_hi = torch.empty(cap, dtype=torch.int32, device=dev)
+        pair_lo = torch.empty(cap, dtype=torch.int32, device=dev)
+        score = torch.empty(cap, dtype=torch.float64 if want == "score" else torch.int32, device=dev)
         count = torch.empty(1, dtype=torch.int64, device=dev)
-        call("mad_match_pairs", C.byref(hi.c), C.byref(lo.c), C.c_double(cc), _ptr(cand_key), _ptr(cand_dot),
-             C.c_uint64(cap), _ptr(count), st)
-        p = _read_counts(count, hi, lo)
+        ws_bytes = _lib.lib.mad_match_pairs_workspace_bytes(hi.rows, lo.rows, cap)
+        ws = torch.empty(ws_bytes, dtype=torch.uint8, device=dev)
+        call("mad_match_pairs_find", C.byref(hi.c), C.byref(lo.c), C.c_double(cc), C.c_uint64(cap), _ptr(count), _ptr(ws), ws_bytes, st)
+
+        def place():
+            call("mad_match_pairs_place", C.byref(hi.c), C.byref(lo.c), C.c_uint64(cap), _ptr(count), _ptr(pair_hi), _ptr(pair_lo),
+                 _ptr(score) if want == "score" else None, _ptr(score) if want != "score" else None, _ptr(ws), ws_bytes, st)
+        p = _read_counts(count, hi, lo, then=place)
         if p >= (1 << 62):
-            raise _lib.MadError("mad_match_pairs: the kernel's internal hand-off timed out (pair list incomplete)")
+            raise _lib.MadError("mad_match_pairs_find: the kernel's internal hand-off timed out (pair list incomplete)")
         if verify and _exact_impl(hi, lo) != 0:
             if want != "score":
                 raise _lib.MadError("match_threshold: entries above 255 need the fp16 or SIMT kernel, which have no want='dot' form")
@@ -525,18 +540,6 @@
             break
         cap = p + p // 8 + 1024
     _PAIR_CAP[key] = max(cap, p + p // 4)
-    pair_hi = torch.empty(max(p, 1), dtype=torch.int32, device=dev)
-    pair_lo = torch.empty(max(p, 1), dtype=torch.int32, device=dev)
-    score = torch.empty(max(p, 1), dtype=torch.float64 if want == "score" else torch.int32, device=dev)
-    if p:
-        ws_bytes = _lib.lib.mad_match_pairs_finish_workspace_bytes(p)
-        ws = torch.empty(ws_bytes, dtype=torch.uint8, device=dev)
-        if want == "score":
-            call("mad_match_pairs_finish", _ptr(cand_key), _ptr(cand_dot), p, hi.rows, lo.rows, _ptr(hi.norm2), _ptr(lo.norm2),
-                 _ptr(pair_hi), _ptr(pair_lo), _ptr(score), _ptr(ws), ws_bytes, st)
-        else:
-            call("mad_match_pairs_finish_dot", _ptr(cand_key), _ptr(cand_dot), p, hi.rows, lo.rows, _ptr(pair_hi), _ptr(pair_lo),
-                 _ptr(score), _ptr(ws), ws_bytes, st)
     return pair_hi[:p], pair_lo[:p], score[:p]
 
 
```
